# JuliaDiff/FiniteDiff.jl

Hardware: NVIDIA H100
Metric: jacobian_nnz_per_s (higher is better)
Workload: dtype f64

## Files before the change

finitediff.jl_b200/csrc/common.cuh:

```cuda
#pragma once
#include <cuda_runtime.h>
#include <stdint.h>

namespace fdb {

template <typename CT> struct ColorTraits;
template <> struct ColorTraits<uint8_t>  { static constexpr uint32_t invalid = 0xFFu; };
template <> struct ColorTraits<uint16_t> { static constexpr uint32_t invalid = 0xFFFFu; };
template <> struct ColorTraits<int32_t>  { static constexpr uint32_t invalid = 0x7FFFFFFFu; };

constexpr int kThreads = 256;

constexpr int kPairsPerThread = 2;
constexpr int kTile = kThreads * 2 * kPairsPerThread;

__device__ __forceinline__ double ld_stream(const double *p) { return __ldcs(p); }
__device__ __forceinline__ void st_stream(double *p, double v) { __stcs(p, v); }
__device__ __forceinline__ double2 ld_stream2(const double *p) { return __ldcs(reinterpret_cast<const double2 *>(p)); }
__device__ __forceinline__ void st_stream2(double *p, double a, double b) {
  __stcs(reinterpret_cast<double2 *>(p), make_double2(a, b));
}

template <typename CT> __device__ __forceinline__ void ld_color_pair(const CT *p, uint32_t &a, uint32_t &b);
template <> __device__ __forceinline__ void ld_color_pair<uint8_t>(const uint8_t *p, uint32_t &a, uint32_t &b) {
  const uint16_t v = __ldcs(reinterpret_cast<const unsigned short *>(p));
  a = v & 0xFFu; b = v >> 8;
}
template <> __device__ __forceinline__ void ld_color_pair<uint16_t>(const uint16_t *p, uint32_t &a, uint32_t &b) {
  const uint32_t v = __ldcs(reinterpret_cast<const unsigned int *>(p));
  a = v & 0xFFFFu; b = v >> 16;
}
template <> __device__ __forceinline__ void ld_color_pair<int32_t>(const int32_t *p, uint32_t &a, uint32_t &b) {
  const int2 v = __ldcs(reinterpret_cast<const int2 *>(p));
  a = (uint32_t)v.x; b = (uint32_t)v.y;
}

__device__ __forceinline__ double warp_sum(double v) {
#pragma unroll
  for (int o = 16; o > 0; o >>= 1) v += __shfl_xor_sync(0xffffffffu, v, o);
  return v;
}

}
```

finitediff.jl_b200/csrc/fdjac_abi.cu:

```cuda
#include "../../include/fdjac_b200.h"

#include <algorithm>
#include <climits>
#include <cstdarg>
#include <cmath>
#include <cfloat>
#include <cstdio>
#include <cstdlib>
#include <cstring>
#include <new>
#include <numeric>
#include <string>
#include <type_traits>
#include <vector>

#include <cub/device/device_radix_sort.cuh>
#include <cub/device/device_scan.cuh>

#include "common.cuh"
#include "kernels_eps.cuh"
#include "kernels_perturb.cuh"
#include "kernels_plan.cuh"
#include "kernels_scatter.cuh"
#include "kernels_staged.cuh"
#include "kernels_jvp.cuh"
#include "kernels_color.cuh"

using namespace fdb;

static thread_local std::string g_err;

static fdb_status fail(fdb_status st, const char *fmt, ...) {
  char buf[512];
  va_list ap;
  va_start(ap, fmt);
  vsnprintf(buf, sizeof buf, fmt, ap);
  va_end(ap);
  g_err = buf;
  return st;
}

#define CU(expr)                                                                                       \
  do {                                                                                                 \
    cudaError_t e__ = (expr);                                                                          \
    if (e__ != cudaSuccess)                                                                            \
      return fail(FDB_ERR_CUDA, "%s failed: %s (%s:%d)", #expr, cudaGetErrorString(e__), __FILE__, __LINE__); \
  } while (0)

#define TRY(expr)                    \
  do {                               \
    fdb_status s__ = (expr);         \
    if (s__ != FDB_OK) return s__;   \
  } while (0)

enum { SP_NONE = 0, SP_CSC = 1, SP_COO = 3, SP_BANDED = 4, SP_JVP = 5, SP_EPS = 6 };

struct DeviceGuard {
  int prev = -1;
  bool ok = false;
  explicit DeviceGuard(int dev) {
    if (cudaGetDevice(&prev) == cudaSuccess) {
      if (prev == dev) ok = true;
      else ok = cudaSetDevice(dev) == cudaSuccess;
    }
  }
  ~DeviceGuard() {
    int cur = -1;
    if (prev >= 0 && cudaGetDevice(&cur) == cudaSuccess && cur != prev) cudaSetDevice(prev);
  }
};

struct GraphKey {
  void *f = nullptr, *ctx = nullptr;
  const void *x = nullptr, *J = nullptr, *fx = nullptr, *f_in = nullptr;
  double relstep = 0, absstep = 0, dir = 0;
  int n_peers = 0;
  long long peer_generation = 0;
  const void *ext_eps = nullptr;
  bool operator==(const GraphKey &o) const {
    return f == o.f && ctx == o.ctx && x == o.x && J == o.J && fx == o.fx && f_in == o.f_in && relstep == o.relstep &&
           absstep == o.absstep && dir == o.dir && n_peers == o.n_peers && peer_generation == o.peer_generation &&
           ext_eps == o.ext_eps;
  }
};

struct fdb_plan {
  int device = 0, sm_count = 132;
  int64_t l2_bytes = 50 << 20;
  int fdtype = FDB_FORWARD, sp_kind = SP_CSC, jkind = FDB_J_CSC_NZVAL;
  int no_drift = 0;
  int rank = 0, world = 1;
  int64_t m = 0, n = 0, E = 0, j_len = 0, ldJ = 0, l = 0, u = 0;
  int32_t C = 0;
  int color_bits = 8;
  bool has_invalid = false;
  void *jcolor = nullptr;
  int32_t *row32 = nullptr;
  void *ecolor = nullptr;
  int64_t *dest = nullptr;
  int32_t *local_of = nullptr;
  int32_t *d_local_colors = nullptr;
  std::vector<int32_t> local_colors, owner;
  double *eps = nullptr, *sumsq = nullptr, *partial = nullptr;
  int eps_blocks = 0;
  int64_t eps_chunk = 0;
  int32_t eps_group = 1;
  const double *ext_eps = nullptr;
  unsigned int *ticket = nullptr;
  bool eps_lists = false;
  int64_t *bucket_start_d = nullptr, *chunk_base_d = nullptr;
  double *eps_list_partial = nullptr;
  int64_t eps_list_max_chunks = 0;
  bool peers_aligned = true;
  bool shared_J = false;
  double *fx_own = nullptr, *Fp = nullptr, *Fm = nullptr, *xp = nullptr, *xm = nullptr;
  int64_t slabs = 0, ldF = 0, ldx = 0, batch = 1, n_groups = 0;
  int64_t pbatch = 1;
  int strategy = 0;
  bool strategy_auto = true;
  bool lists_resident = false;
  struct Tunables {
    bool no_staged = false, no_eps_lists = false, no_eps_overlap = false, cm_prefetch = false, force_overlap = false;
    bool no_fx_cm = false, force_fx_cm = false, no_pack = false;
    int hi_stream = -1;
    int reverse = 3;
    int cm_slab_stream = 1;
    int eps_depth = 2;
    int cols_depth = 0, cols_gx = 64;
    int stages = 2;
    char staged_variant[3] = {'6', 'n', 0};
  } tune;
  bool double_buffer = false;
  cudaStream_t side = nullptr;
  cudaEvent_t ev_f[2] = {nullptr, nullptr}, ev_scat[2] = {nullptr, nullptr};
  cudaEvent_t ev_fork = nullptr, ev_eps = nullptr;
  int32_t *colptr32 = nullptr, *cols_by_color = nullptr;
  int32_t *cm_row = nullptr;
  void *cm_slot = nullptr;
  int64_t *cm_start = nullptr;
  double *fx_cm = nullptr;
  std::vector<int64_t> cm_start_h;
  int64_t cm_invalid_end = 0;
  uint16_t *row16 = nullptr;
  int32_t *tile_w0 = nullptr;
  int32_t stage_W = 0;
  bool staged = false, stage_packed = false;
  std::vector<int64_t> bucket_start;
  int lanes = 1;
  double mean_row_jump = 0.0;
  double **d_peers = nullptr;
  int n_peers = 0;
  int64_t col_begin = 0, col_end = 0;
  double *eps_cols = nullptr;
  cudaStream_t hstream = nullptr;
  double *h_dx = nullptr, *h_dJ = nullptr, *h_dfx = nullptr, *h_dfin = nullptr;
  std::vector<void *> allocs;
  size_t device_bytes = 0;
  fdb_counters_t cnt{};
  int64_t alg_bytes = 0;
  int64_t last_eps_count = 0;
  bool complex_entry = false;
  bool use_graph = false;
  cudaStream_t cstream = nullptr;
  cudaGraphExec_t graph_exec = nullptr;
  GraphKey graph_key;
  fdb_counters_t graph_delta{};
  long long peer_generation = 0;
  bool timing = false;
  std::vector<std::pair<cudaEvent_t, cudaEvent_t>> ev_pending, ev_pool;

  fdb_status alloc(void **p, size_t bytes) {
    if (bytes == 0) bytes = 16;
    cudaError_t e = cudaMalloc(p, bytes);
    if (e != cudaSuccess) {
      *p = nullptr;
      return fail(FDB_ERR_NOMEM, "cudaMalloc(%zu bytes) failed: %s", bytes, cudaGetErrorString(e));
    }
    allocs.push_back(*p);
    device_bytes += bytes;
    return FDB_OK;
  }
  template <typename T> fdb_status alloc_t(T **p, size_t count) { return alloc((void **)p, count * sizeof(T)); }
  int grid(int64_t items, int per_block = kThreads, int waves = 8) const {
    int64_t b = (items + per_block - 1) / per_block;
    const int64_t cap = (int64_t)sm_count * waves;
    if (b > cap) b = cap;
    if (b < 1) b = 1;
    return (int)b;
  }
};

struct I64View {
  const int64_t *d = nullptr;
  int64_t *owned = nullptr;
  ~I64View() { if (owned) cudaFree(owned); }
};

static fdb_status view_i64(const int64_t *p, int64_t count, I64View &v) {
  if (!p || count <= 0) { v.d = nullptr; return FDB_OK; }
  cudaPointerAttributes at{};
  cudaError_t e = cudaPointerGetAttributes(&at, p);
  if (e != cudaSuccess) { cudaGetLastError(); at.type = cudaMemoryTypeUnregistered; }
  if (at.type == cudaMemoryTypeDevice || at.type == cudaMemoryTypeManaged) { v.d = p; return FDB_OK; }
  CU(cudaMalloc((void **)&v.owned, (size_t)count * sizeof(int64_t)));
  CU(cudaMemcpy(v.owned, p, (size_t)count * sizeof(int64_t), cudaMemcpyHostToDevice));
  v.d = v.owned;
  return FDB_OK;
}

static fdb_status check_device(const fdb_plan_opts *o, int *dev) {
  int count = 0;
  cudaError_t e = cudaGetDeviceCount(&count);
  if (e != cudaSuccess || count <= 0) {
    cudaGetLastError();
    return fail(FDB_ERR_NO_DEVICE, "no CUDA device available (%s): libfdjac_b200 has no CPU fallback",
                e == cudaSuccess ? "device count 0" : cudaGetErrorString(e));
  }
  int d = 0;
  if (!o || o->use_current_device || o->device < 0) { CU(cudaGetDevice(&d)); }
  else d = o->device;
  if (d >= count) return fail(FDB_ERR_INVALID, "device %d out of range (%d devices)", d, count);
  *dev = d;
  return FDB_OK;
}

template <typename F> static fdb_status dispatch_ct(int bits, F &&fn) {
  if (bits == 8) return fn((uint8_t)0);
  if (bits == 16) return fn((uint16_t)0);
  return fn((int32_t)0);
}

static const char *plan_err_text(uint32_t e) {
  if (e & kErrColptr) return "colptr is not a valid CSC column pointer (must start at 1, be non-decreasing, end at nnz+1)";
  if (e & kErrRowRange) return "row index outside 1..m";
  if (e & kErrColRange) return "column index outside 1..n";
  if (e & kErrSlotRange) return "slot outside 1..j_len";
  if (e & kErrMissingInJ) return "a sparsity entry is absent from J's CSC pattern (the reference would insert a new stored entry; unsupported)";
  return "invalid pattern";
}

static fdb_status setup_colors(fdb_plan *P, const int64_t *colorvec , I64View &cv) {
  const int64_t n = P->n;
  TRY(view_i64(colorvec, n, cv));
  long long mx = n, mn = n > 0 ? 1 : 0;
  if (cv.d && n > 0) {
    long long *d_mm = nullptr;
    CU(cudaMalloc((void **)&d_mm, 2 * sizeof(long long)));
    long long init[2] = {LLONG_MIN, LLONG_MAX};
    CU(cudaMemcpy(d_mm, init, sizeof init, cudaMemcpyHostToDevice));
    color_minmax<<<P->grid(n), kThreads>>>(cv.d, n, d_mm, d_mm + 1);
    long long out[2];
    cudaError_t e = cudaMemcpy(out, d_mm, sizeof out, cudaMemcpyDeviceToHost);
    cudaFree(d_mm);
    if (e != cudaSuccess) return fail(FDB_ERR_CUDA, "colour min/max failed: %s", cudaGetErrorString(e));
    mx = out[0];
    mn = out[1];
  }
  if (n == 0) mx = 0;
  if (mx < 0) mx = 0;
  if (mx > 0x7FFFFFF0LL) return fail(FDB_ERR_UNSUPPORTED, "maximum(colorvec) = %lld exceeds 2^31", mx);
  P->C = (int32_t)mx;
  P->has_invalid = n > 0 && mn < 1;
  P->color_bits = mx <= 255 ? 8 : (mx <= 65535 ? 16 : 32);
  TRY(P->alloc(&P->jcolor, (size_t)std::max<int64_t>(n, 1) * (P->color_bits / 8)));
  if (n > 0) {
    uint32_t *d_flags = nullptr;
    const bool window_path = P->C > kEpsRegColors;
    if (window_path) {
      CU(cudaMalloc((void **)&d_flags, sizeof(uint32_t)));
      CU(cudaMemset(d_flags, 0, sizeof(uint32_t)));
    }
    fdb_status st = dispatch_ct(P->color_bits, [&](auto tag) -> fdb_status {
      using CT = decltype(tag);
      convert_colors<CT><<<P->grid(n), kThreads>>>(cv.d, n, (CT *)P->jcolor);
      if (window_path) color_lane_conflicts<CT><<<P->grid(n), kThreads>>>((const CT *)P->jcolor, n, P->C, d_flags);
      CU(cudaGetLastError());
      return FDB_OK;
    });
    if (st == FDB_OK && window_path) {
      uint32_t flags = 0;
      cudaError_t e = cudaMemcpy(&flags, d_flags, sizeof flags, cudaMemcpyDeviceToHost);
      if (e != cudaSuccess) st = fail(FDB_ERR_CUDA, "colour conflict flags: %s", cudaGetErrorString(e));
      P->eps_group = 1;
      for (int lg = 1; lg <= 5 && !(flags & (1u << lg)); ++lg) P->eps_group = 1 << lg;
    }
    if (d_flags) cudaFree(d_flags);
    if (st != FDB_OK) return st;
  }
  return FDB_OK;
}

static fdb_status alloc_eps_buffers(fdb_plan *P) {
  const int32_t C = P->C;
  TRY(P->alloc_t(&P->eps, std::max<int32_t>(C, 1)));
  TRY(P->alloc_t(&P->sumsq, std::max<int32_t>(C, 1)));
  {
    int64_t nb = (P->n + 2047) / 2048;
    nb = std::max<int64_t>(1, std::min<int64_t>(nb, (int64_t)P->sm_count * (C <= 256 ? 8 : 6)));
    P->eps_blocks = (int)nb;
    int64_t chunk = (P->n + nb - 1) / nb;
    P->eps_chunk = (std::max<int64_t>(chunk, 1) + 31) & ~(int64_t)31;
    const int64_t stride = C <= kEpsRegColors ? kEpsRegColors : std::min<int64_t>(C, kEpsWindow);
    TRY(P->alloc_t(&P->partial, (size_t)nb * stride));
    TRY(P->alloc_t(&P->ticket, 4));
    CU(cudaMemset(P->ticket, 0, 16));
  }

  return FDB_OK;
}

static fdb_status finish_colored_plan(fdb_plan *P, const fdb_plan_opts *o, const std::vector<unsigned long long> &count) {
  const int32_t C = P->C;
  P->owner.assign(C, 0);
  const int world = P->world;
  if (world > 1) {
    if (o && o->partition == 1) {
      std::vector<int32_t> order(C);
      std::iota(order.begin(), order.end(), 0);
      std::stable_sort(order.begin(), order.end(), [&](int32_t a, int32_t b) { return count[a] > count[b]; });
      std::vector<unsigned long long> load(world, 0);
      for (int32_t k : order) {
        int best = 0;
        for (int r = 1; r < world; ++r) if (load[r] < load[best]) best = r;
        P->owner[k] = best;
        load[best] += count[k] + 1;
      }
    } else {
      for (int32_t k = 0; k < C; ++k) P->owner[k] = k % world;
    }
  }
  std::vector<int32_t> local_of(C, -1);
  P->local_colors.clear();
  for (int32_t k = 0; k < C; ++k)
    if (P->owner[k] == P->rank) { local_of[k] = (int32_t)P->local_colors.size(); P->local_colors.push_back(k); }
  const int64_t n_local = (int64_t)P->local_colors.size();
  TRY(P->alloc_t(&P->local_of, std::max<int32_t>(C, 1)));
  TRY(P->alloc_t(&P->d_local_colors, std::max<int64_t>(n_local, 1)));
  if (C > 0) CU(cudaMemcpy(P->local_of, local_of.data(), (size_t)C * 4, cudaMemcpyHostToDevice));
  if (n_local > 0) CU(cudaMemcpy(P->d_local_colors, P->local_colors.data(), (size_t)n_local * 4, cudaMemcpyHostToDevice));

  TRY(alloc_eps_buffers(P));

  const bool central = P->fdtype == FDB_CENTRAL;
  const int64_t cw = P->fdtype == FDB_COMPLEX ? 2 : 1;
  P->ldF = (P->m + 1) & ~(int64_t)1;
  P->ldx = (P->n + 1) & ~(int64_t)1;
  if (P->ldF < 2) P->ldF = 2;
  if (P->ldx < 2) P->ldx = 2;
  int64_t budget = (o && o->scratch_bytes > 0) ? o->scratch_bytes : (int64_t)8 << 30;
  const int64_t per_slab = 8 * cw * P->ldF * (central ? 2 : 1);
  int64_t slabs = std::max<int64_t>(1, budget / per_slab);
  slabs = std::min<int64_t>(slabs, std::max<int64_t>(n_local, 1));
  if (P->sp_kind == SP_CSC && P->strategy == 0 && P->strategy_auto && slabs < n_local) P->strategy = 1;
  if (P->strategy == 1 && !P->lists_resident) {
    const int64_t l2_slabs = std::max<int64_t>(1, P->l2_bytes * 2 / 5 / per_slab);
    slabs = std::min<int64_t>(slabs, l2_slabs);
  }
  if (P->strategy == 1) slabs = std::min<int64_t>(slabs, kCmMaxGroup);
  P->slabs = slabs;
  P->n_groups = n_local == 0 ? 0 : (n_local + slabs - 1) / slabs;
  int64_t batch = (o && o->max_batch > 1) ? o->max_batch : 1;
  batch = std::min<int64_t>(batch, slabs);
  P->batch = batch;
  int64_t pbatch = std::max<int64_t>(batch, std::min<int64_t>(kPerturbMaxPoints, std::max<int64_t>(n_local, 1)));
  while (pbatch > batch && pbatch * 8 * cw * P->ldx * (central ? 2 : 1) > budget / 8) --pbatch;
  P->pbatch = pbatch;
  P->double_buffer = false;
  if (P->tune.force_overlap && P->sp_kind == SP_CSC && P->strategy == 1 && (int64_t)P->local_colors.size() > slabs) P->double_buffer = true;
  const size_t nbuf = P->double_buffer ? 2 : 1;
  CU(cudaStreamCreateWithFlags(&P->side, cudaStreamNonBlocking));
  CU(cudaEventCreateWithFlags(&P->ev_fork, cudaEventDisableTiming));
  CU(cudaEventCreateWithFlags(&P->ev_eps, cudaEventDisableTiming));
  if (P->double_buffer) {
    for (int b = 0; b < 2; ++b) {
      CU(cudaEventCreateWithFlags(&P->ev_f[b], cudaEventDisableTiming));
      CU(cudaEventCreateWithFlags(&P->ev_scat[b], cudaEventDisableTiming));
    }
  }
  TRY(P->alloc_t(&P->fx_own, (size_t)P->ldF));
  TRY(P->alloc_t(&P->Fp, nbuf * (size_t)slabs * P->ldF * cw));
  TRY(P->alloc_t(&P->xp, (size_t)pbatch * P->ldx * cw));
  if (central) {
    TRY(P->alloc_t(&P->Fm, nbuf * (size_t)slabs * P->ldF));
    TRY(P->alloc_t(&P->xm, (size_t)pbatch * P->ldx));
  }
  return FDB_OK;
}

static fdb_status build_color_lists(fdb_plan *P) {
  const int64_t n = P->n;
  const int32_t C = P->C;
  if (!P->cols_by_color) TRY(P->alloc_t(&P->cols_by_color, (size_t)std::max<int64_t>(n, 1)));
  if (n > 0) {
    uint32_t *k_in = nullptr, *k_out = nullptr;
    int32_t *v_in = nullptr;
    void *d_tmp = nullptr;
    size_t tmp_bytes = 0;
    auto cleanup = [&]() { cudaFree(k_in); cudaFree(k_out); cudaFree(v_in); cudaFree(d_tmp); };
    cudaError_t e = cudaMalloc((void **)&k_in, (size_t)n * 4);
    if (e == cudaSuccess) e = cudaMalloc((void **)&k_out, (size_t)n * 4);
    if (e == cudaSuccess) e = cudaMalloc((void **)&v_in, (size_t)n * 4);
    if (e == cudaSuccess) {
      dispatch_ct(P->color_bits, [&](auto tag) -> fdb_status {
        using CT = decltype(tag);
        color_sort_keys<CT><<<P->grid(n), kThreads>>>((const CT *)P->jcolor, n, C, k_in, v_in);
        return FDB_OK;
      });
      int end_bit = 1;
      while (end_bit < 32 && ((uint64_t)1 << end_bit) <= (uint64_t)C) ++end_bit;
      e = cub::DeviceRadixSort::SortPairs(nullptr, tmp_bytes, k_in, k_out, v_in, P->cols_by_color, (int)n, 0, end_bit);
      if (e == cudaSuccess) e = cudaMalloc(&d_tmp, tmp_bytes ? tmp_bytes : 16);
      if (e == cudaSuccess) e = cub::DeviceRadixSort::SortPairs(d_tmp, tmp_bytes, k_in, k_out, v_in, P->cols_by_color, (int)n, 0, end_bit);
      if (e == cudaSuccess) e = cudaDeviceSynchronize();
    }
    cleanup();
    if (e != cudaSuccess) return fail(FDB_ERR_CUDA, "column lists: %s", cudaGetErrorString(e));
  }
  if (C > kEpsRegColors && C <= (1 << 22) && n > 0) {
    std::vector<int64_t> cb((size_t)C + 1, 0);
    int64_t maxc = 1;
    for (int32_t k = 0; k < C; ++k) {
      const int64_t len = P->bucket_start[(size_t)k + 1] - P->bucket_start[(size_t)k];
      const int64_t nc = (len + kEpsListChunk - 1) / kEpsListChunk;
      cb[(size_t)k + 1] = cb[(size_t)k] + nc;
      maxc = std::max(maxc, nc);
    }
    TRY(P->alloc_t(&P->bucket_start_d, (size_t)C + 2));
    TRY(P->alloc_t(&P->chunk_base_d, (size_t)C + 1));
    TRY(P->alloc_t(&P->eps_list_partial, (size_t)std::max<int64_t>(cb[(size_t)C], 1)));
    CU(cudaMemcpy(P->bucket_start_d, P->bucket_start.data(), ((size_t)C + 2) * 8, cudaMemcpyHostToDevice));
    CU(cudaMemcpy(P->chunk_base_d, cb.data(), ((size_t)C + 1) * 8, cudaMemcpyHostToDevice));
    P->eps_list_max_chunks = maxc;
    P->eps_lists = true;
  }
  return FDB_OK;
}

static fdb_status bucket_offsets(fdb_plan *P, const unsigned long long *d_bucket_counts) {
  const int32_t C = P->C;
  std::vector<unsigned long long> bc((size_t)C + 1, 0);
  CU(cudaMemcpy(bc.data(), d_bucket_counts, ((size_t)C + 1) * 8, cudaMemcpyDeviceToHost));
  P->bucket_start.assign((size_t)C + 2, 0);
  for (int32_t k = 0; k <= C; ++k) P->bucket_start[(size_t)k + 1] = P->bucket_start[(size_t)k] + (int64_t)bc[(size_t)k];
  return FDB_OK;
}

__global__ void __launch_bounds__(kThreads)
cm_gather_cols(const int32_t *__restrict__ cols_by_color, const int64_t *__restrict__ src_start ,
               const int64_t *__restrict__ dst_start , int64_t nseg, int32_t *__restrict__ list_cols) {
  for (int64_t sgm = blockIdx.x; sgm < nseg; sgm += gridDim.x) {
    const int64_t s0 = src_start[sgm], d0 = dst_start[sgm], cnt = dst_start[sgm + 1] - d0;
    for (int64_t i = threadIdx.x; i < cnt; i += kThreads) list_cols[d0 + i] = cols_by_color[s0 + i];
  }
}

static fdb_status build_cm_lists(fdb_plan *P, const std::vector<unsigned long long> &count ) {
  const int64_t n_local = (int64_t)P->local_colors.size();
  const int32_t C = P->C;
  const bool zero_bucket = P->rank == 0 && P->bucket_start[(size_t)C + 1] > P->bucket_start[(size_t)C];
  const int64_t nseg = n_local + (zero_bucket ? 1 : 0);
  std::vector<int64_t> src(std::max<int64_t>(nseg, 1), 0), dst((size_t)nseg + 1, 0);
  P->cm_start_h.assign((size_t)n_local + 1, 0);
  unsigned long long valid_total = 0;
  for (int32_t k = 0; k < C; ++k) valid_total += count[(size_t)k];
  for (int64_t li = 0; li < n_local; ++li) {
    const int32_t k = P->local_colors[(size_t)li];
    src[(size_t)li] = P->bucket_start[(size_t)k];
    dst[(size_t)li + 1] = dst[(size_t)li] + (P->bucket_start[(size_t)k + 1] - P->bucket_start[(size_t)k]);
    P->cm_start_h[(size_t)li + 1] = P->cm_start_h[(size_t)li] + (int64_t)count[(size_t)k];
  }
  int64_t e_local = P->cm_start_h[(size_t)n_local];
  P->cm_invalid_end = e_local;
  if (zero_bucket) {
    src[(size_t)n_local] = P->bucket_start[(size_t)C];
    dst[(size_t)n_local + 1] = dst[(size_t)n_local] + (P->bucket_start[(size_t)C + 1] - P->bucket_start[(size_t)C]);
    e_local += P->E - (int64_t)valid_total;
    P->cm_invalid_end = e_local;
  }
  const int64_t ncols = dst[(size_t)nseg];
  TRY(P->alloc_t(&P->cm_start, (size_t)n_local + 1));
  CU(cudaMemcpy(P->cm_start, P->cm_start_h.data(), ((size_t)n_local + 1) * 8, cudaMemcpyHostToDevice));
  TRY(P->alloc_t(&P->cm_row, (size_t)std::max<int64_t>(e_local, 1)));
  {
    const bool want = P->n_groups > 1 || P->tune.force_fx_cm;
    if (P->fdtype == FDB_FORWARD && e_local > 0 && want && !P->tune.no_fx_cm) TRY(P->alloc_t(&P->fx_cm, (size_t)e_local));
  }
  const bool wide = P->dest != nullptr;
  TRY(P->alloc(&P->cm_slot, (size_t)std::max<int64_t>(e_local, 1) * (wide ? 8 : 4)));
  if (ncols == 0 || e_local == 0) return FDB_OK;
  int64_t *d_src = nullptr, *d_dst = nullptr;
  int32_t *list_cols = nullptr, *list_cnt = nullptr, *list_off = nullptr;
  void *d_tmp = nullptr;
  size_t tmp_bytes = 0;
  auto cleanup = [&]() {
    cudaFree(d_src); cudaFree(d_dst); cudaFree(list_cols); cudaFree(list_cnt); cudaFree(list_off); cudaFree(d_tmp);
  };
#define CM_CU(expr) do { cudaError_t e__ = (expr); if (e__ != cudaSuccess) { cleanup(); \
    return fail(FDB_ERR_CUDA, "%s failed: %s", #expr, cudaGetErrorString(e__)); } } while (0)
  CM_CU(cudaMalloc((void **)&d_src, (size_t)nseg * 8));
  CM_CU(cudaMalloc((void **)&d_dst, ((size_t)nseg + 1) * 8));
  CM_CU(cudaMalloc((void **)&list_cols, (size_t)ncols * 4));
  CM_CU(cudaMalloc((void **)&list_cnt, (size_t)ncols * 4));
  CM_CU(cudaMalloc((void **)&list_off, (size_t)ncols * 4));
  CM_CU(cudaMemcpy(d_src, src.data(), (size_t)nseg * 8, cudaMemcpyHostToDevice));
  CM_CU(cudaMemcpy(d_dst, dst.data(), ((size_t)nseg + 1) * 8, cudaMemcpyHostToDevice));
  cm_gather_cols<<<(int)std::min<int64_t>(nseg, (int64_t)P->sm_count * 16), kThreads>>>(P->cols_by_color, d_src, d_dst, nseg, list_cols);
  cm_column_counts<<<P->grid(ncols), kThreads>>>(list_cols, ncols, P->colptr32, list_cnt);
  CM_CU(cub::DeviceScan::ExclusiveSum(nullptr, tmp_bytes, list_cnt, list_off, (int)ncols));
  CM_CU(cudaMalloc(&d_tmp, tmp_bytes ? tmp_bytes : 16));
  CM_CU(cub::DeviceScan::ExclusiveSum(d_tmp, tmp_bytes, list_cnt, list_off, (int)ncols));
  {
    const int lanes = P->lanes;
    const int64_t blocks = (ncols + (kThreads / lanes) - 1) / (kThreads / lanes);
    const int grid = (int)std::max<int64_t>(1, std::min<int64_t>(blocks, (int64_t)P->sm_count * 16));
    if (wide) cm_expand<int64_t><<<grid, kThreads>>>(list_cols, list_off, ncols, P->colptr32, P->row32, P->dest, lanes, P->cm_row, (int64_t *)P->cm_slot);
    else cm_expand<int32_t><<<grid, kThreads>>>(list_cols, list_off, ncols, P->colptr32, P->row32, nullptr, lanes, P->cm_row, (int32_t *)P->cm_slot);
  }
  int32_t last_off = 0, last_cnt = 0;
  CM_CU(cudaMemcpy(&last_off, list_off + (ncols - 1), 4, cudaMemcpyDeviceToHost));
  CM_CU(cudaMemcpy(&last_cnt, list_cnt + (ncols - 1), 4, cudaMemcpyDeviceToHost));
  CM_CU(cudaDeviceSynchronize());
#undef CM_CU
  cleanup();
  if ((int64_t)last_off + last_cnt != e_local)
    return fail(FDB_ERR_INVALID, "internal: colour-major list holds %lld entries, expected %lld", (long long)last_off + last_cnt,
                (long long)e_local);
  return FDB_OK;
}

static fdb_status try_stage_plan(fdb_plan *P) {
  P->staged = false;
  if (P->tune.no_staged) return FDB_OK;
  if (P->sp_kind != SP_CSC || P->dest != nullptr || P->strategy != 0 || P->world != 1 || P->n_groups != 1) return FDB_OK;
  if (P->fdtype == FDB_COMPLEX || P->C < 1) return FDB_OK;
  const int nwin = P->fdtype == FDB_CENTRAL ? 2 * P->C : P->C + 1;
  const int64_t ntiles = P->E / kTile;
  if (nwin > kStageMaxWin || ntiles < 1) return FDB_OK;
  unsigned int *d_span = nullptr;
  TRY(P->alloc_t(&d_span, 1));
  CU(cudaMemset(d_span, 0, 4));
  TRY(P->alloc_t(&P->tile_w0, (size_t)ntiles));
  TRY(P->alloc_t(&P->row16, (size_t)ntiles * kTile));
  const int pgrid = (int)std::min<int64_t>(ntiles, (int64_t)P->sm_count * 16);
  stage_prepare<uint8_t><<<pgrid, kThreads>>>(P->row32, ntiles, P->tile_w0, P->row16, d_span, nullptr, P->C);
  unsigned int span = 0;
  CU(cudaMemcpy(&span, d_span, 4, cudaMemcpyDeviceToHost));
  const int64_t W = ((int64_t)span + 1) & ~(int64_t)1;
  P->stage_packed = P->C <= 14 && W <= 4096 && span > 0 && !P->tune.no_pack;
  if (P->stage_packed) {
    TRY(dispatch_ct(P->color_bits, [&](auto tag) -> fdb_status {
      using CT = decltype(tag);
      stage_prepare<CT><<<pgrid, kThreads>>>(P->row32, ntiles, P->tile_w0, P->row16, d_span, (const CT *)P->ecolor, P->C);
      CU(cudaGetLastError());
      return FDB_OK;
    }));
    CU(cudaDeviceSynchronize());
  }
  const size_t smem = (size_t)2 * nwin * W * 8 + 2 * kStagesMax * 8 + (size_t)P->C * 8;
  if (span == 0 || span > 65535 || smem > (size_t)kStageMaxSmem) return FDB_OK;
  P->stage_W = (int32_t)W;
  P->staged = true;
  return FDB_OK;
}

static fdb_status read_plan_err(uint32_t *d_err, const char *what) {
  uint32_t h = 0;
  CU(cudaMemcpy(&h, d_err, 4, cudaMemcpyDeviceToHost));
  const uint32_t hard = h & ~(uint32_t)(kErrPatternDiff | kErrRowOrder);
  if (hard == kErrMissingInJ) return fail(FDB_ERR_UNSUPPORTED, "%s: %s", what, plan_err_text(hard));
  if (hard) return fail(FDB_ERR_INVALID, "%s: %s", what, plan_err_text(hard));
  return FDB_OK;
}

static bool env_is(const char *name, char c) {
  const char *v = getenv(name);
  return v && v[0] == c;
}

static void read_tunables(fdb_plan *P) {
  auto &t = P->tune;
  t.no_staged = env_is("FDB_NO_STAGED", '1');
  t.no_eps_lists = env_is("FDB_NO_EPS_LISTS", '1');
  t.no_eps_overlap = env_is("FDB_NO_EPS_OVERLAP", '1');
  t.cm_prefetch = env_is("FDB_CM_PREFETCH", '1');
  t.force_overlap = env_is("FDB_FORCE_OVERLAP", '1');
  t.no_fx_cm = env_is("FDB_NO_FX_CM", '1');
  t.force_fx_cm = env_is("FDB_FORCE_FX_CM", '1');
  t.no_pack = env_is("FDB_NO_PACK", '1');
  if (const char *hs = getenv("FDB_HI_STREAM")) t.hi_stream = hs[0] == '1' ? 1 : 0;
  if (const char *v = getenv("FDB_REVERSE")) { if (v[0] >= '0' && v[0] <= '3') t.reverse = v[0] - '0'; }
  if (env_is("FDB_CM_HINT", '0')) t.cm_slab_stream = 0;
  if (env_is("FDB_STAGES", '3')) t.stages = 3;
  if (env_is("FDB_EPS_DEPTH", '1')) t.eps_depth = 1;
  if (env_is("FDB_COLS_DEPTH", '4')) t.cols_depth = 4;
  if (env_is("FDB_COLS_DEPTH", '2')) t.cols_depth = 2;
  if (env_is("FDB_COLS_DEPTH", '1')) t.cols_depth = 1;
  if (const char *v = getenv("FDB_COLS_GX")) { const int g = atoi(v); if (g >= 1 && g <= 4096) t.cols_gx = g; }
  if (const char *v = getenv("FDB_STAGED_VARIANT")) {
    if (v[0]) { t.staged_variant[0] = v[0]; t.staged_variant[1] = v[1] ? v[1] : 'n'; }
  }
}

static fdb_status new_plan(fdb_plan **out, const fdb_plan_opts *o, int64_t m, int64_t n) {
  if (!out) return fail(FDB_ERR_INVALID, "plan output pointer is NULL");
  *out = nullptr;
  if (m < 0 || n < 0) return fail(FDB_ERR_INVALID, "negative dimensions m=%lld n=%lld", (long long)m, (long long)n);
  if (m > 0x7FFFFFF0LL || n > 0x7FFFFFF0LL) return fail(FDB_ERR_UNSUPPORTED, "m, n must be < 2^31");
  if (o && o->fdtype != FDB_FORWARD && o->fdtype != FDB_CENTRAL && o->fdtype != FDB_COMPLEX)
    return fail(FDB_ERR_UNSUPPORTED, "Unrecognized fdtype: valid values are forward (0), central (1) and complex (2)");
  int dev = 0;
  TRY(check_device(o, &dev));
  fdb_plan *P = new (std::nothrow) fdb_plan();
  if (!P) return fail(FDB_ERR_NOMEM, "out of host memory");
  P->device = dev;
  P->m = m;
  P->n = n;
  P->fdtype = o ? o->fdtype : FDB_FORWARD;
  P->no_drift = o ? o->no_drift : 0;
  P->use_graph = o && o->use_graph != 0;
  P->shared_J = o && o->shared_j != 0;
  read_tunables(P);
  P->world = (o && o->world > 1) ? o->world : 1;
  P->rank = (o && o->world > 1) ? o->rank : 0;
  if (P->rank < 0 || P->rank >= P->world) {
    const int bad_rank = P->rank, bad_world = P->world;
    delete P;
    return fail(FDB_ERR_INVALID, "rank %d outside world %d", bad_rank, bad_world);
  }
  cudaDeviceProp prop;
  cudaError_t e = cudaGetDeviceProperties(&prop, dev);
  if (e != cudaSuccess) { delete P; return fail(FDB_ERR_CUDA, "cudaGetDeviceProperties: %s", cudaGetErrorString(e)); }
  P->sm_count = prop.multiProcessorCount;
  P->l2_bytes = prop.l2CacheSize;
  *out = P;
  return FDB_OK;
}

static void free_plan(fdb_plan *P) {
  if (!P) return;
  DeviceGuard g(P->device);
  for (void *p : P->allocs) cudaFree(p);
  for (auto &ev : P->ev_pending) { cudaEventDestroy(ev.first); cudaEventDestroy(ev.second); }
  for (auto &ev : P->ev_pool) { cudaEventDestroy(ev.first); cudaEventDestroy(ev.second); }
  if (P->hstream) cudaStreamDestroy(P->hstream);
  if (P->side) cudaStreamDestroy(P->side);
  for (int b = 0; b < 2; ++b) { if (P->ev_f[b]) cudaEventDestroy(P->ev_f[b]); if (P->ev_scat[b]) cudaEventDestroy(P->ev_scat[b]); }
  if (P->ev_fork) cudaEventDestroy(P->ev_fork);
  if (P->ev_eps) cudaEventDestroy(P->ev_eps);
  if (P->graph_exec) cudaGraphExecDestroy(P->graph_exec);
  if (P->cstream) cudaStreamDestroy(P->cstream);
  delete P;
}

#define PLAN_TRY(expr)                                   \
  do {                                                   \
    fdb_status s__ = (expr);                             \
    if (s__ != FDB_OK) { free_plan(P); *plan = nullptr; return s__; } \
  } while (0)

static inline void resolve_steps(int fdtype, double &relstep, double &absstep) {
  if (std::isnan(relstep)) relstep = fdb_default_relstep(fdtype);
  if (std::isnan(absstep)) absstep = relstep;
}

extern "C" {

int fdb_abi_version(void) { return FDB_ABI_VERSION; }
const char *fdb_last_error(void) { return g_err.c_str(); }
int fdb_device_count(void) {
  int c = 0;
  if (cudaGetDeviceCount(&c) != cudaSuccess) { cudaGetLastError(); return 0; }
  return c;
}

double fdb_default_relstep(int fdtype) {
  if (fdtype == FDB_FORWARD) return sqrt(DBL_EPSILON);
  if (fdtype == FDB_CENTRAL) return cbrt(DBL_EPSILON);
  return 1.0;
}
double fdb_compute_epsilon(int fdtype, double x, double relstep, double absstep, double dir) {
  const double a = relstep * fabs(x);
  const double e = a > absstep ? a : absstep;
  return fdtype == FDB_FORWARD ? e * dir : e;
}

fdb_status fdb_plan_create_csc(fdb_plan **plan, int64_t m, int64_t n, const int64_t *colptr, const int64_t *rowval,
                               int jkind, const int64_t *j_colptr, const int64_t *j_rowval, int64_t ldJ,
                               const int64_t *colorvec, const fdb_plan_opts *opts) {
  fdb_plan *P = nullptr;
  TRY(new_plan(plan, opts, m, n));
  P = *plan;
  DeviceGuard g(P->device);
  if (!colptr) { free_plan(P); *plan = nullptr; return fail(FDB_ERR_INVALID, "colptr is NULL"); }
  if (jkind != FDB_J_CSC_NZVAL && jkind != FDB_J_DENSE) {
    free_plan(P); *plan = nullptr;
    return fail(FDB_ERR_INVALID, "CSC sparsity supports J kinds CSC_NZVAL and DENSE");
  }
  P->sp_kind = SP_CSC;
  P->jkind = jkind;
  I64View cp, rv, cv, jcp, jrv;
  PLAN_TRY(view_i64(colptr, n + 1, cp));
  int64_t last = 1;
  {
    cudaError_t e = cudaMemcpy(&last, cp.d + n, 8, cudaMemcpyDeviceToHost);
    if (e != cudaSuccess) { free_plan(P); *plan = nullptr; return fail(FDB_ERR_CUDA, "reading colptr[n]: %s", cudaGetErrorString(e)); }
  }
  const int64_t nnz = last - 1;
  if (nnz < 0 || nnz > 0x7FFFFFF0LL) { free_plan(P); *plan = nullptr; return fail(FDB_ERR_UNSUPPORTED, "nnz=%lld unsupported (must be in [0, 2^31))", (long long)nnz); }
  if (nnz > 0 && !rowval) { free_plan(P); *plan = nullptr; return fail(FDB_ERR_INVALID, "rowval is NULL"); }
  P->E = nnz;
  PLAN_TRY(view_i64(rowval, nnz, rv));
  PLAN_TRY(setup_colors(P, colorvec, cv));

  uint32_t *d_err = nullptr;
  unsigned long long *d_cnt = nullptr;
  PLAN_TRY(P->alloc_t(&d_err, 1));
  PLAN_TRY(P->alloc_t(&d_cnt, std::max<int32_t>(P->C, 1)));
  cudaMemset(d_err, 0, 4);
  cudaMemset(d_cnt, 0, (size_t)std::max<int32_t>(P->C, 1) * 8);
  PLAN_TRY(P->alloc_t(&P->row32, std::max<int64_t>(nnz, 4)));
  PLAN_TRY(P->alloc(&P->ecolor, (size_t)std::max<int64_t>(nnz, 4) * (P->color_bits / 8) + 16));

  bool same_pattern = true;
  bool other_csc = false;
  if (jkind == FDB_J_CSC_NZVAL && j_colptr && j_rowval && (j_colptr != colptr || j_rowval != rowval)) {
    PLAN_TRY(view_i64(j_colptr, n + 1, jcp));
    int64_t jlast = 1;
    {
      cudaError_t e = cudaMemcpy(&jlast, jcp.d + n, 8, cudaMemcpyDeviceToHost);
      if (e != cudaSuccess) { free_plan(P); *plan = nullptr; return fail(FDB_ERR_CUDA, "reading J.colptr[n]: %s", cudaGetErrorString(e)); }
    }
    if (jlast < 1 || jlast - 1 > 0x7FFFFFF0LL) { free_plan(P); *plan = nullptr; return fail(FDB_ERR_INVALID, "J.colptr[n+1]=%lld is not a valid CSC end pointer", (long long)jlast); }
    const int64_t jnnz = jlast - 1;
    PLAN_TRY(view_i64(j_rowval, jnnz, jrv));
    if (jnnz != nnz) same_pattern = false;
    else {
      compare_i64<<<P->grid(n + 1), kThreads>>>(cp.d, jcp.d, n + 1, d_err);
      if (nnz > 0) compare_i64<<<P->grid(nnz), kThreads>>>(rv.d, jrv.d, nnz, d_err);
      uint32_t h = 0;
      cudaMemcpy(&h, d_err, 4, cudaMemcpyDeviceToHost);
      same_pattern = !(h & kErrPatternDiff);
      cudaMemset(d_err, 0, 4);
    }
    other_csc = !same_pattern;
    P->j_len = jnnz;
  } else if (jkind == FDB_J_CSC_NZVAL) {
    P->j_len = nnz;
  } else {
    if (ldJ < m) { free_plan(P); *plan = nullptr; return fail(FDB_ERR_INVALID, "ldJ=%lld < m=%lld", (long long)ldJ, (long long)m); }
    P->ldJ = ldJ;
    P->j_len = ldJ * n;
  }
  const bool need_dest = jkind == FDB_J_DENSE || other_csc;
  int32_t *col32 = nullptr;
  if (need_dest) {
    PLAN_TRY(P->alloc_t(&col32, std::max<int64_t>(nnz, 1)));
    PLAN_TRY(P->alloc_t(&P->dest, std::max<int64_t>(nnz, 1)));
  }
  validate_colptr<<<P->grid(n + 1), kThreads>>>(cp.d, n, nnz, d_err);
  PLAN_TRY(read_plan_err(d_err, "CSC sparsity"));
  if (other_csc) {
    validate_colptr<<<P->grid(n + 1), kThreads>>>(jcp.d, n, P->j_len, d_err);
    PLAN_TRY(read_plan_err(d_err, "J's CSC pattern"));
  }
  if (nnz > 0) {
    PLAN_TRY(dispatch_ct(P->color_bits, [&](auto tag) -> fdb_status {
      using CT = decltype(tag);
      const size_t hsm = P->C <= kPlanSmemColors ? (size_t)std::max<int32_t>(P->C, 1) * sizeof(unsigned int) : 0;
      expand_csc<CT><<<P->grid(nnz), kThreads, hsm>>>(cp.d, rv.d, m, n, nnz, (const CT *)P->jcolor, P->C, P->row32,
                                                 (CT *)P->ecolor, col32, d_cnt, d_err);
      CU(cudaGetLastError());
      return FDB_OK;
    }));
    if (jkind == FDB_J_DENSE) dest_dense_from_rc<<<P->grid(nnz), kThreads>>>(P->row32, col32, nnz, ldJ, P->dest);
    else if (other_csc) dest_other_csc<<<P->grid(nnz), kThreads>>>(P->row32, col32, nnz, jcp.d, jrv.d, P->dest, d_err);
  }
  PLAN_TRY(read_plan_err(d_err, "CSC sparsity"));
  std::vector<unsigned long long> cnt(std::max<int32_t>(P->C, 1), 0);
  if (P->C > 0) {
    cudaError_t e = cudaMemcpy(cnt.data(), d_cnt, (size_t)P->C * 8, cudaMemcpyDeviceToHost);
    if (e != cudaSuccess) { free_plan(P); *plan = nullptr; return fail(FDB_ERR_CUDA, "colour counts: %s", cudaGetErrorString(e)); }
  }
  {
    const int32_t C = P->C;
    unsigned long long *d_bucket = nullptr, *d_jump = nullptr;
    PLAN_TRY(P->alloc_t(&d_bucket, (size_t)C + 2));
    PLAN_TRY(P->alloc_t(&d_jump, 1));
    cudaMemset(d_bucket, 0, ((size_t)C + 2) * 8);
    cudaMemset(d_jump, 0, 8);
    PLAN_TRY(P->alloc_t(&P->colptr32, (size_t)n + 1));
    PLAN_TRY(P->alloc_t(&P->cols_by_color, (size_t)std::max<int64_t>(n, 1)));
    PLAN_TRY(dispatch_ct(P->color_bits, [&](auto tag) -> fdb_status {
      using CT = decltype(tag);
      colptr32_and_count<CT><<<P->grid(n + 1), kThreads>>>(cp.d, n, (const CT *)P->jcolor, C, P->colptr32, d_bucket);
      CU(cudaGetLastError());
      return FDB_OK;
    }));
    std::vector<unsigned long long> bc((size_t)C + 1, 0);
    {
      cudaError_t e = cudaMemcpy(bc.data(), d_bucket, ((size_t)C + 1) * 8, cudaMemcpyDeviceToHost);
      if (e != cudaSuccess) { free_plan(P); *plan = nullptr; return fail(FDB_ERR_CUDA, "column buckets: %s", cudaGetErrorString(e)); }
    }
    P->bucket_start.assign((size_t)C + 2, 0);
    for (int32_t k = 0; k <= C; ++k) P->bucket_start[(size_t)k + 1] = P->bucket_start[(size_t)k] + (int64_t)bc[(size_t)k];
    PLAN_TRY(build_color_lists(P));
    if (nnz > 1) {
      row_jump_sum<<<P->grid(nnz), kThreads>>>(P->row32, nnz, d_jump);
      unsigned long long js = 0;
      cudaMemcpy(&js, d_jump, 8, cudaMemcpyDeviceToHost);
      P->mean_row_jump = (double)js / (double)(nnz - 1);
    }
    int lanes = 1;
    const double avg = n > 0 ? (double)nnz / (double)n : 1.0;
    while (lanes < 32 && lanes < avg) lanes *= 2;
    P->lanes = lanes;
    const int want = opts ? opts->strategy : 0;
    bool per_color = P->world > 1;
    if (want == 1) per_color = false;
    if (want == 2 || want == 3) per_color = true;
    P->lists_resident = want == 3;
    if (want == 0 && P->world == 1 && P->mean_row_jump > 4096.0 && C >= 16 && 16 * P->m <= P->l2_bytes) {
      per_color = true;
      P->lists_resident = true;
    }
    P->strategy = per_color ? 1 : 0;
    P->strategy_auto = want == 0;
  }
  PLAN_TRY(finish_colored_plan(P, opts, cnt));
  if (P->strategy == 1) PLAN_TRY(build_cm_lists(P, cnt));
  PLAN_TRY(try_stage_plan(P));
  P->alg_bytes = 32 * nnz + 16 * n + 8;
  {
    cudaError_t e = cudaDeviceSynchronize();
    if (e != cudaSuccess) { free_plan(P); *plan = nullptr; return fail(FDB_ERR_CUDA, "plan build: %s", cudaGetErrorString(e)); }
  }
  return FDB_OK;
}

fdb_status fdb_plan_create_coo(fdb_plan **plan, int64_t m, int64_t n, int64_t nnz, const int64_t *rows_index,
                               const int64_t *cols_index, int jkind, const int64_t *slots, int64_t ldJ_or_jlen,
                               const int64_t *colorvec, const fdb_plan_opts *opts) {
  fdb_plan *P = nullptr;
  TRY(new_plan(plan, opts, m, n));
  P = *plan;
  DeviceGuard g(P->device);
  if (nnz < 0 || nnz > 0x7FFFFFF0LL) { free_plan(P); *plan = nullptr; return fail(FDB_ERR_UNSUPPORTED, "nnz=%lld unsupported", (long long)nnz); }
  if (nnz > 0 && (!rows_index || !cols_index)) { free_plan(P); *plan = nullptr; return fail(FDB_ERR_INVALID, "rows_index/cols_index NULL"); }
  if (jkind != FDB_J_DENSE && jkind != FDB_J_SLOTS) { free_plan(P); *plan = nullptr; return fail(FDB_ERR_INVALID, "COO sparsity supports J kinds DENSE and SLOTS"); }
  if (jkind == FDB_J_SLOTS && nnz > 0 && !slots) { free_plan(P); *plan = nullptr; return fail(FDB_ERR_INVALID, "slots is NULL"); }
  if (jkind == FDB_J_DENSE && ldJ_or_jlen < m) { free_plan(P); *plan = nullptr; return fail(FDB_ERR_INVALID, "ldJ < m"); }
  P->sp_kind = SP_COO;
  P->jkind = jkind;
  P->E = nnz;
  if (jkind == FDB_J_DENSE) { P->ldJ = ldJ_or_jlen; P->j_len = ldJ_or_jlen * n; }
  else P->j_len = ldJ_or_jlen;
  I64View rv, cvw, sv, cv;
  PLAN_TRY(view_i64(rows_index, nnz, rv));
  PLAN_TRY(view_i64(cols_index, nnz, cvw));
  if (jkind == FDB_J_SLOTS) PLAN_TRY(view_i64(slots, nnz, sv));
  PLAN_TRY(setup_colors(P, colorvec, cv));
  uint32_t *d_err = nullptr;
  unsigned long long *d_cnt = nullptr;
  PLAN_TRY(P->alloc_t(&d_err, 1));
  PLAN_TRY(P->alloc_t(&d_cnt, std::max<int32_t>(P->C, 1)));
  cudaMemset(d_err, 0, 4);
  cudaMemset(d_cnt, 0, (size_t)std::max<int32_t>(P->C, 1) * 8);
  PLAN_TRY(P->alloc_t(&P->row32, std::max<int64_t>(nnz, 4)));
  PLAN_TRY(P->alloc(&P->ecolor, (size_t)std::max<int64_t>(nnz, 4) * (P->color_bits / 8) + 16));
  PLAN_TRY(P->alloc_t(&P->dest, std::max<int64_t>(nnz, 1)));
  if (nnz > 0) {
    PLAN_TRY(dispatch_ct(P->color_bits, [&](auto tag) -> fdb_status {
      using CT = decltype(tag);
      const size_t hsm = P->C <= kPlanSmemColors ? (size_t)std::max<int32_t>(P->C, 1) * sizeof(unsigned int) : 0;
      prepare_coo<CT><<<P->grid(nnz), kThreads, hsm>>>(rv.d, cvw.d, jkind == FDB_J_SLOTS ? sv.d : nullptr, nnz, m, n, P->ldJ,
                                                  P->j_len, (const CT *)P->jcolor, P->C, P->row32, (CT *)P->ecolor,
                                                  P->dest, d_cnt, d_err);
      CU(cudaGetLastError());
      return FDB_OK;
    }));
  }
  PLAN_TRY(read_plan_err(d_err, "COO sparsity"));
  std::vector<unsigned long long> cnt(std::max<int32_t>(P->C, 1), 0);
  if (P->C > 0) cudaMemcpy(cnt.data(), d_cnt, (size_t)P->C * 8, cudaMemcpyDeviceToHost);
  PLAN_TRY(finish_colored_plan(P, opts, cnt));
  P->alg_bytes = 32 * nnz + 16 * n + 8;
  cudaError_t e = cudaDeviceSynchronize();
  if (e != cudaSuccess) { free_plan(P); *plan = nullptr; return fail(FDB_ERR_CUDA, "plan build: %s", cudaGetErrorString(e)); }
  return FDB_OK;
}

fdb_status fdb_plan_create_banded(fdb_plan **plan, int64_t m, int64_t n, int64_t l, int64_t u, int jkind, int64_t ldJ,
                                  const int64_t *colorvec, const fdb_plan_opts *opts) {
  fdb_plan *P = nullptr;
  TRY(new_plan(plan, opts, m, n));
  P = *plan;
  DeviceGuard g(P->device);
  if (jkind != FDB_J_BAND && jkind != FDB_J_DENSE) { free_plan(P); *plan = nullptr; return fail(FDB_ERR_INVALID, "banded sparsity supports J kinds BAND and DENSE"); }
  if (l + u + 1 < 1 || l < -n || u < -m) { free_plan(P); *plan = nullptr; return fail(FDB_ERR_INVALID, "invalid bandwidths l=%lld u=%lld", (long long)l, (long long)u); }
  if (jkind == FDB_J_DENSE && ldJ < m) { free_plan(P); *plan = nullptr; return fail(FDB_ERR_INVALID, "ldJ < m"); }
  P->sp_kind = SP_BANDED;
  P->jkind = jkind;
  P->l = l;
  P->u = u;
  P->ldJ = ldJ;
  P->j_len = jkind == FDB_J_BAND ? (l + u + 1) * n : ldJ * n;
  I64View cv;
  PLAN_TRY(setup_colors(P, colorvec, cv));
  unsigned long long *d_cnt = nullptr;
  PLAN_TRY(P->alloc_t(&d_cnt, std::max<int32_t>(P->C, 1)));
  cudaMemset(d_cnt, 0, (size_t)std::max<int32_t>(P->C, 1) * 8);
  if (n > 0 && P->C > 0) {
    PLAN_TRY(dispatch_ct(P->color_bits, [&](auto tag) -> fdb_status {
      using CT = decltype(tag);
      count_band_colors<CT><<<P->grid(n), kThreads>>>((const CT *)P->jcolor, m, n, l, u, P->C, d_cnt);
      CU(cudaGetLastError());
      return FDB_OK;
    }));
  }
  std::vector<unsigned long long> cnt(std::max<int32_t>(P->C, 1), 0);
  if (P->C > 0) cudaMemcpy(cnt.data(), d_cnt, (size_t)P->C * 8, cudaMemcpyDeviceToHost);
  unsigned long long total = 0;
  for (auto c : cnt) total += c;
  P->E = (int64_t)total;
  PLAN_TRY(finish_colored_plan(P, opts, cnt));
  P->alg_bytes = 8 * (int64_t)total + 16 * m * (int64_t)P->C;
  cudaError_t e = cudaDeviceSynchronize();
  if (e != cudaSuccess) { free_plan(P); *plan = nullptr; return fail(FDB_ERR_CUDA, "plan build: %s", cudaGetErrorString(e)); }
  return FDB_OK;
}

static fdb_status create_dense(fdb_plan **plan, int64_t m, int64_t n, int64_t ldJ, int64_t ncols, const fdb_plan_opts *opts) {
  fdb_plan *P = nullptr;
  TRY(new_plan(plan, opts, m, n));
  P = *plan;
  DeviceGuard g(P->device);
  if (ldJ < m) { free_plan(P); *plan = nullptr; return fail(FDB_ERR_INVALID, "ldJ < m"); }
  P->sp_kind = SP_NONE;
  P->jkind = FDB_J_DENSE;
  P->ldJ = ldJ;
  const int64_t per = (ncols + P->world - 1) / P->world;
  P->col_begin = std::min<int64_t>(ncols, per * P->rank);
  P->col_end = std::min<int64_t>(ncols, P->col_begin + per);
  const int64_t ncl = P->col_end - P->col_begin;
  P->j_len = ldJ * ncl;
  P->E = m * ncl;
  P->C = (int32_t)n;
  const bool central = P->fdtype == FDB_CENTRAL;
  P->ldF = std::max<int64_t>(2, (m + 1) & ~(int64_t)1);
  P->ldx = std::max<int64_t>(2, (n + 1) & ~(int64_t)1);
  int64_t batch = (opts && opts->max_batch > 1) ? opts->max_batch : 1;
  int64_t budget = (opts && opts->scratch_bytes > 0) ? opts->scratch_bytes : (int64_t)8 << 30;
  const int64_t cw = P->fdtype == FDB_COMPLEX ? 2 : 1;
  const int64_t per_point = 8 * cw * (P->ldx + P->ldF * (central ? 2 : 1));
  batch = std::max<int64_t>(1, std::min<int64_t>(batch, budget / per_point));
  batch = std::min<int64_t>(batch, std::max<int64_t>(ncl, 1));
  batch = std::min<int64_t>(batch, 65535);
  P->batch = batch;
  P->slabs = batch;
  P->n_groups = ncl == 0 ? 0 : (ncl + batch - 1) / batch;
  PLAN_TRY(P->alloc_t(&P->fx_own, (size_t)P->ldF));
  PLAN_TRY(P->alloc_t(&P->Fp, (size_t)batch * P->ldF * cw));
  if (central) PLAN_TRY(P->alloc_t(&P->Fm, (size_t)batch * P->ldF));
  PLAN_TRY(P->alloc_t(&P->xp, (size_t)batch * P->ldx * cw));
  PLAN_TRY(P->alloc_t(&P->eps_cols, (size_t)std::max<int64_t>(ncl, 1)));
  P->alg_bytes = 24 * m * ncl;
  return FDB_OK;
}

fdb_status fdb_plan_create_dense(fdb_plan **plan, int64_t m, int64_t n, int64_t ldJ, const fdb_plan_opts *opts) {
  return create_dense(plan, m, n, ldJ, n, opts);
}

fdb_status fdb_plan_create_dense_colorvec(fdb_plan **plan, int64_t m, int64_t n, int64_t ldJ, const int64_t *colorvec,
                                          const fdb_plan_opts *opts) {
  if (!plan) return fail(FDB_ERR_INVALID, "plan output pointer is NULL");
  *plan = nullptr;
  if (!colorvec) return create_dense(plan, m, n, ldJ, n, opts);
  if (n < 0 || m < 0) return fail(FDB_ERR_INVALID, "negative dimensions");
  int dev = 0;
  TRY(check_device(opts, &dev));
  DeviceGuard g(dev);
  long long mx = 0;
  if (n > 0) {
    I64View cv;
    TRY(view_i64(colorvec, n, cv));
    long long *d_mm = nullptr;
    CU(cudaMalloc((void **)&d_mm, 2 * sizeof(long long)));
    const long long init[2] = {LLONG_MIN, LLONG_MAX};
    cudaMemcpy(d_mm, init, sizeof init, cudaMemcpyHostToDevice);
    const int blocks = (int)std::max<int64_t>(1, std::min<int64_t>((n + kThreads - 1) / kThreads, 132 * 8));
    color_minmax<<<blocks, kThreads>>>(cv.d, n, d_mm, d_mm + 1);
    long long out[2] = {0, 0};
    const cudaError_t e = cudaMemcpy(out, d_mm, sizeof out, cudaMemcpyDeviceToHost);
    cudaFree(d_mm);
    if (e != cudaSuccess) return fail(FDB_ERR_CUDA, "colour maximum failed: %s", cudaGetErrorString(e));
    mx = out[0];
  }
  if (mx > n) return fail(FDB_ERR_INVALID, "sparsity=nothing: maximum(colorvec)=%lld indexes x beyond length(x)=%lld "
                                           "(BoundsError in the reference, jacobians.jl:549)", mx, (long long)n);
  return create_dense(plan, m, n, ldJ, mx < 0 ? 0 : (int64_t)mx, opts);
}

fdb_status fdb_plan_destroy(fdb_plan *plan) {
  free_plan(plan);
  return FDB_OK;
}

fdb_status fdb_plan_info(const fdb_plan *P, fdb_plan_info_t *info) {
  if (!P || !info) return fail(FDB_ERR_INVALID, "NULL argument");
  memset(info, 0, sizeof *info);
  info->m = P->m;
  info->n = P->n;
  info->n_entries = P->E;
  info->j_len = P->j_len;
  info->n_colors = P->C;
  const int64_t n_local = P->sp_kind == SP_NONE ? P->col_end - P->col_begin : (int64_t)P->local_colors.size();
  info->n_local_colors = n_local;
  info->n_groups = P->n_groups;
  info->slabs = P->slabs;
  info->fcalls_per_jacobian = P->fdtype == FDB_CENTRAL ? 2 * n_local : (P->fdtype == FDB_COMPLEX ? n_local : 1 + n_local);
  info->device_bytes = (int64_t)P->device_bytes;
  info->fdtype = P->fdtype;
  info->jkind = P->jkind;
  info->sp_kind = P->sp_kind;
  info->color_bits = P->color_bits;
  info->alg_bytes_scatter = P->alg_bytes;
  info->strategy = P->strategy;
  info->lanes = P->lanes;
  info->mean_row_jump = P->mean_row_jump;
  info->staged = P->staged ? 1 : 0;
  info->lists_resident = P->lists_resident ? 1 : 0;
  {
    const int64_t ct = P->color_bits / 8;
    const int64_t slabs_read = P->fdtype == FDB_CENTRAL ? 2 : 1;
    const int64_t fx_once = P->fdtype == FDB_FORWARD ? 8 * P->m : 0;
    if (P->sp_kind == SP_CSC || P->sp_kind == SP_COO) {
      if (P->sp_kind == SP_CSC && P->strategy == 1) {
        const int64_t e_local = P->cm_start_h.empty() ? 0 : P->cm_start_h.back();
        info->moved_bytes_scatter = e_local * (4 + (P->dest ? 8 : 4) + 8 * slabs_read + 8) + fx_once + (P->fx_cm ? e_local * (4 + 8 + 8) : 0);
      } else {
        const int64_t C = std::max<int32_t>(P->C, 1);
        const int64_t owned = P->world > 1 ? P->E * (int64_t)P->local_colors.size() / C : P->E;
        info->moved_bytes_scatter = P->E * (4 + ct) * std::max<int64_t>(P->n_groups, 1) + owned * (8 * slabs_read + 8 + (P->dest ? 8 : 0)) + fx_once;
        if (P->staged)
          info->moved_bytes_scatter = P->E * (2 + (P->stage_packed ? 0 : ct) + 8) + 8 * P->m * (int64_t)(P->fdtype == FDB_CENTRAL ? 2 * P->C : P->C + 1);
      }
    } else {
      info->moved_bytes_scatter = P->alg_bytes;
    }
  }
  return FDB_OK;
}

fdb_status fdb_plan_counters(const fdb_plan *P, fdb_counters_t *out) {
  if (!P || !out) return fail(FDB_ERR_INVALID, "NULL argument");
  *out = P->cnt;
  return FDB_OK;
}

fdb_status fdb_plan_dense_range(const fdb_plan *P, int64_t *b, int64_t *e) {
  if (!P || !b || !e) return fail(FDB_ERR_INVALID, "NULL argument");
  *b = P->col_begin;
  *e = P->col_end;
  return FDB_OK;
}

fdb_status fdb_plan_color_owner(const fdb_plan *P, int32_t *owner_out, int64_t cap) {
  if (!P || !owner_out) return fail(FDB_ERR_INVALID, "NULL argument");
  if (P->sp_kind == SP_NONE) return fail(FDB_ERR_INVALID, "dense plans partition columns by range");
  if (cap < (int64_t)P->owner.size()) return fail(FDB_ERR_INVALID, "owner_out too small");
  std::copy(P->owner.begin(), P->owner.end(), owner_out);
  return FDB_OK;
}

fdb_status fdb_plan_get_eps(fdb_plan *P, double *h_eps, int64_t cap, void *stream) {
  if (!P || !h_eps) return fail(FDB_ERR_INVALID, "NULL argument");
  DeviceGuard g(P->device);
  const int64_t count = P->sp_kind == SP_NONE ? P->col_end - P->col_begin : P->C;
  if (cap < count) return fail(FDB_ERR_INVALID, "h_eps too small (%lld < %lld)", (long long)cap, (long long)count);
  const double *src = P->sp_kind == SP_NONE ? P->eps_cols : P->eps;
  if (count > 0) {
    CU(cudaMemcpyAsync(h_eps, src, (size_t)count * 8, cudaMemcpyDeviceToHost, (cudaStream_t)stream));
    CU(cudaStreamSynchronize((cudaStream_t)stream));
  }
  return FDB_OK;
}

fdb_status fdb_plan_enable_timing(fdb_plan *P, int enable) {
  if (!P) return fail(FDB_ERR_INVALID, "NULL plan");
  P->timing = enable != 0;
  return FDB_OK;
}

fdb_status fdb_plan_read_timing(fdb_plan *P, double *scatter_ms, int64_t *scatter_launches) {
  if (!P || !scatter_ms || !scatter_launches) return fail(FDB_ERR_INVALID, "NULL argument");
  DeviceGuard g(P->device);
  double total = 0.0;
  int64_t count = 0;
  for (auto &ev : P->ev_pending) {
    CU(cudaEventSynchronize(ev.second));
    float ms = 0.f;
    CU(cudaEventElapsedTime(&ms, ev.first, ev.second));
    total += ms;
    count += 1;
    P->ev_pool.push_back(ev);
  }
  P->ev_pending.clear();
  *scatter_ms = total;
  *scatter_launches = count;
  return FDB_OK;
}

fdb_status fdb_plan_set_peers(fdb_plan *P, int n_peers, double *const *peer_J) {
  if (!P) return fail(FDB_ERR_INVALID, "NULL plan");
  if (n_peers < 0 || n_peers > 64) return fail(FDB_ERR_INVALID, "n_peers out of range");
  if (P->sp_kind == SP_NONE || P->sp_kind == SP_BANDED)
    return fail(FDB_ERR_UNSUPPORTED, "peer stores are implemented for the entry-driven (CSC / COO) scatters");
  DeviceGuard g(P->device);
  if (!P->d_peers) TRY(P->alloc_t(&P->d_peers, 64));
  if (n_peers > 0) CU(cudaMemcpy(P->d_peers, peer_J, (size_t)n_peers * sizeof(double *), cudaMemcpyHostToDevice));
  P->n_peers = n_peers;
  P->peer_generation += 1;
  P->peers_aligned = true;
  for (int i = 0; i < n_peers; ++i)
    if (reinterpret_cast<uintptr_t>(peer_J[i]) & 15) P->peers_aligned = false;
  return FDB_OK;
}

}

struct ScatterTimer {
  fdb_plan *P;
  cudaStream_t s;
  std::pair<cudaEvent_t, cudaEvent_t> ev{nullptr, nullptr};
  ScatterTimer(fdb_plan *p, cudaStream_t st) : P(p), s(st) {
    if (!P->timing) return;
    if (!P->ev_pool.empty()) { ev = P->ev_pool.back(); P->ev_pool.pop_back(); }
    else { cudaEventCreate(&ev.first); cudaEventCreate(&ev.second); }
    cudaEventRecord(ev.first, s);
  }
  ~ScatterTimer() {
    if (!P->timing || !ev.first) return;
    cudaEventRecord(ev.second, s);
    P->ev_pending.push_back(ev);
  }
};

static fdb_status zero_J(const fdb_plan *P, double *J, cudaStream_t s) {
  if (P->jkind == FDB_J_DENSE && P->ldJ > P->m) {
    const int64_t ncols = P->sp_kind == SP_NONE ? P->col_end - P->col_begin : P->n;
    if (P->m > 0 && ncols > 0)
      CU(cudaMemset2DAsync(J, (size_t)P->ldJ * 8, 0, (size_t)P->m * 8, (size_t)ncols, s));
    return FDB_OK;
  }
  CU(cudaMemsetAsync(J, 0, (size_t)P->j_len * 8, s));
  return FDB_OK;
}

static fdb_status call_f(fdb_plan *P, fdb_fn f, void *ctx, double *fx, const double *x, int64_t batch, cudaStream_t s) {
  const int rc = f(ctx, fx, x, batch, P->ldF, P->ldx, (void *)s);
  P->cnt.f_invocations += 1;
  P->cnt.f_points += batch;
  if (rc != 0) return fail(FDB_ERR_CALLBACK, "user f! returned %d", rc);
  return FDB_OK;
}

template <typename K>
static int resident_grid(const fdb_plan *P, K kernel, size_t dyn_smem, int64_t work_blocks) {
  int per_sm = 0;
  if (cudaOccupancyMaxActiveBlocksPerMultiprocessor(&per_sm, kernel, kThreads, dyn_smem) != cudaSuccess || per_sm < 1) {
    cudaGetLastError();
    per_sm = 4;
  }
  int64_t g = (int64_t)P->sm_count * per_sm;
  if (g > work_blocks) g = work_blocks;
  if (g < 1) g = 1;
  return (int)g;
}

template <typename CT>
static fdb_status run_eps(fdb_plan *P, const double *x, double relstep, double absstep, double dir, cudaStream_t s) {
  const int32_t C = P->C;
  if (C <= 0) return FDB_OK;
  if (P->fdtype == FDB_COMPLEX) {
    fill_value<<<(C + kThreads - 1) / kThreads, kThreads, 0, s>>>(P->eps, C, DBL_EPSILON);
    P->cnt.kernel_launches += 1;
    CU(cudaGetLastError());
    return FDB_OK;
  }
  EpsParams prm{P->fdtype == FDB_CENTRAL ? 1 : 0, relstep, absstep, dir};
  if (P->eps_lists) {
    if (!P->tune.no_eps_lists) {
      dim3 grid((unsigned)std::min<int64_t>(P->eps_list_max_chunks, 1024), (unsigned)std::min<int32_t>(C, 65535));
      color_sumsq_lists<<<grid, kThreads, 0, s>>>(x, P->cols_by_color, P->bucket_start_d, P->chunk_base_d, C, P->eps_list_partial);
      finalize_eps_lists<<<(int)std::min<int64_t>(((int64_t)C * 32 + kThreads - 1) / kThreads, (int64_t)P->sm_count * 8), kThreads, 0, s>>>(
          P->eps_list_partial, P->chunk_base_d, C, prm, P->eps, P->sumsq);
      P->cnt.kernel_launches += 2;
      CU(cudaGetLastError());
      return FDB_OK;
    }
  }
  if (C <= kEpsRegColors) {
    const int64_t ntiles = (P->n + kTile - 1) / kTile;
    const int aligned = (reinterpret_cast<uintptr_t>(x) & 15) == 0;
    auto go = [&](auto kern) {
      const int grid = std::min(resident_grid(P, kern, 0, ntiles), P->eps_blocks);
      kern<<<grid, kThreads, 0, s>>>(x, (const CT *)P->jcolor, P->n, aligned, C, prm, P->partial, P->ticket, P->eps, P->sumsq);
    };
    if (C <= 4) { if (P->tune.eps_depth == 2) go(color_sumsq_reg<CT, 4, 2>); else go(color_sumsq_reg<CT, 4, 1>); }
    else { if (P->tune.eps_depth == 2) go(color_sumsq_reg<CT, 8, 2>); else go(color_sumsq_reg<CT, 8, 1>); }
    P->cnt.kernel_launches += 1;
  } else {
    for (int32_t k0 = 0; k0 < C; k0 += kEpsWindow) {
      const int32_t W = std::min<int32_t>(kEpsWindow, C - k0);
      color_sumsq_win<CT><<<P->eps_blocks, kThreads, (size_t)kEpsWarps * W * sizeof(double), s>>>(
          x, (const CT *)P->jcolor, P->n, P->eps_chunk, k0, W, P->eps_group, P->partial);
      finalize_eps<<<(W * 32 + kThreads - 1) / kThreads, kThreads, 0, s>>>(P->partial, P->eps_blocks, W, k0, W, prm,
                                                                        P->eps, P->sumsq);
      P->cnt.kernel_launches += 2;
    }
  }
  CU(cudaGetLastError());
  return FDB_OK;
}

template <typename CT, int MODE>
static fdb_status run_colored(fdb_plan *P, fdb_fn f, void *ctx, const double *x, double *J, double *fx,
                              const double *f_in, double relstep, double absstep, double dir, cudaStream_t s) {
  constexpr bool CENTRAL = MODE == kCentral;
  constexpr bool COMPLEX = MODE == kComplex;
  const int64_t sF = COMPLEX ? 2 * P->ldF : P->ldF, sX = COMPLEX ? 2 * P->ldx : P->ldx;
  const int64_t n_local = (int64_t)P->local_colors.size();
  const bool ident = P->dest == nullptr && P->sp_kind != SP_BANDED;
  const bool band_data = P->sp_kind == SP_BANDED && P->jkind == FDB_J_BAND;
  const bool self_defining = (ident || band_data) && n_local > 0;
  if (!self_defining && P->n_peers == 0 && !P->shared_J && P->j_len > 0) TRY(zero_J(P, J, s));
  bool eps_beside_fx = MODE == kForward && !f_in && !P->ext_eps && P->side && P->ev_fork && P->C > 0;
  if (P->tune.no_eps_overlap) eps_beside_fx = false;
  if (P->ext_eps) {
    if (P->C > 0) CU(cudaMemcpyAsync(P->eps, P->ext_eps, (size_t)P->C * 8, cudaMemcpyDeviceToDevice, s));
  } else if (eps_beside_fx) {
    CU(cudaEventRecord(P->ev_fork, s));
    CU(cudaStreamWaitEvent(P->side, P->ev_fork, 0));
    TRY(run_eps<CT>(P, x, relstep, absstep, dir, P->side));
    CU(cudaEventRecord(P->ev_eps, P->side));
  } else {
    TRY(run_eps<CT>(P, x, relstep, absstep, dir, s));
  }
  const double *vfx = nullptr;
  if (MODE == kForward) {
    if (f_in) vfx = f_in;
    else { TRY(call_f(P, f, ctx, fx, x, 1, s)); vfx = fx; }
  }
  if (eps_beside_fx) CU(cudaStreamWaitEvent(s, P->ev_eps, 0));
  if (MODE == kForward && P->sp_kind == SP_CSC && P->strategy == 1 && P->fx_cm && n_local > 0) {
    const int64_t cnt = P->cm_start_h[(size_t)n_local];
    if (cnt > 0) {
      const int grid = (int)std::max<int64_t>(1, std::min<int64_t>((cnt + kThreads * 4 - 1) / (kThreads * 4), (int64_t)P->sm_count * 16));
      ScatterTimer tm(P, s);
      gather_fx_cm<<<grid, kThreads, 0, s>>>(P->cm_row, vfx, cnt, P->fx_cm);
      P->cnt.kernel_launches += 1;
    }
  }
  auto perturb_window = [&](int64_t li0, int64_t kc) -> fdb_status {
      for (int64_t q0 = 0; q0 < kc; q0 += kPerturbMaxPoints) {
        PerturbArgs pa{};
        pa.x = x; pa.jcolor = P->jcolor; pa.eps = P->eps;
        pa.xp = P->xp + q0 * sX; pa.xm = CENTRAL ? P->xm + q0 * sX : nullptr;
        pa.n = P->n; pa.ldx = sX; pa.C = P->C; pa.drift = P->no_drift ? 0 : 1;
        pa.reverse = (P->tune.reverse >> 1) & 1;
        pa.kcount = (int32_t)std::min<int64_t>(kPerturbMaxPoints, kc - q0);
        for (int32_t q = 0; q < pa.kcount; ++q) pa.k[q] = P->local_colors[(size_t)(li0 + q0 + q)];
        pa.aligned = ((reinterpret_cast<uintptr_t>(x) | reinterpret_cast<uintptr_t>(P->xp) |
                       reinterpret_cast<uintptr_t>(P->xm)) & 15) == 0 && (P->ldx & 1) == 0;
        const size_t sm = P->C <= kPerturbSmemColors ? (size_t)P->C * sizeof(double) : 0;
        const int64_t tiles = (P->n + kTile - 1) / kTile;
        if (COMPLEX) {
          if (pa.kcount == 1) perturb_complex<CT, 1><<<P->grid(P->n), kThreads, 0, s>>>(pa);
          else perturb_complex<CT, kPerturbMaxPoints><<<P->grid(P->n), kThreads, 0, s>>>(pa);
        } else {
          constexpr int kPerturbGridOver = 16;
          auto over = [&](int g) { return (int)std::max<int64_t>(1, std::min<int64_t>((int64_t)g * kPerturbGridOver, tiles)); };
          if (pa.kcount == 1)
            perturb_colors<CT, CENTRAL, 1><<<over(resident_grid(P, perturb_colors<CT, CENTRAL, 1>, sm, tiles)), kThreads, sm, s>>>(pa);
          else
            perturb_colors<CT, CENTRAL, kPerturbMaxPoints><<<over(resident_grid(P, perturb_colors<CT, CENTRAL, kPerturbMaxPoints>, sm, tiles)), kThreads, sm, s>>>(pa);
        }
        P->cnt.kernel_launches += 1;
      }
      return FDB_OK;
  };

  const bool overlap = P->double_buffer && P->side != nullptr;
  const double *Fp_g = P->Fp, *Fm_g = P->Fm;
  cudaStream_t ss = s;
  auto scatter_lists = [&](int64_t g, int64_t l0, int64_t G) -> fdb_status {
    const bool wide = P->dest != nullptr;
    if (g == 0 && P->rank == 0 && P->cm_invalid_end > P->cm_start_h[(size_t)n_local]) {
      const int64_t z0 = P->cm_start_h[(size_t)n_local], z1 = P->cm_invalid_end;
      const int grid = (int)std::max<int64_t>(1, std::min<int64_t>((z1 - z0 + kThreads - 1) / kThreads, (int64_t)P->sm_count * 8));
      if (wide) zero_slots<int64_t><<<grid, kThreads, 0, ss>>>(P->cm_slot, z0, z1, J, P->d_peers, P->n_peers);
      else zero_slots<int32_t><<<grid, kThreads, 0, ss>>>(P->cm_slot, z0, z1, J, P->d_peers, P->n_peers);
      P->cnt.kernel_launches += 1;
    }
    if (G <= 0) return FDB_OK;
    const int64_t total = P->cm_start_h[(size_t)(l0 + G)] - P->cm_start_h[(size_t)l0];
    if (total == 0) return FDB_OK;
    CmArgs a{};
    a.row = P->cm_row; a.slot = P->cm_slot; a.seg_start = P->cm_start; a.local_colors = P->d_local_colors;
    a.fx = vfx; a.Fp = Fp_g; a.Fm = Fm_g; a.eps = P->eps; a.J = J; a.peers = P->d_peers; a.n_peers = P->n_peers;
    a.fx_cm = MODE == kForward ? P->fx_cm : nullptr;
    a.l0 = (int32_t)l0; a.G = (int32_t)G; a.ldF = sF;
    a.m = COMPLEX ? 2 * P->m : P->m;
    a.prefetch_next = (G > 1 && P->tune.cm_prefetch) ? 1 : 0;
    a.slab_stream = P->tune.cm_slab_stream;
    const int64_t tiles = (total + kCmTile - 1) / kCmTile;
    ScatterTimer tm(P, ss);
    if (wide) {
      const int grid = resident_grid(P, diff_scatter_cm<MODE, int64_t>, 0, tiles);
      diff_scatter_cm<MODE, int64_t><<<grid, kThreads, 0, ss>>>(a);
    } else {
      const int grid = resident_grid(P, diff_scatter_cm<MODE, int32_t>, 0, tiles);
      diff_scatter_cm<MODE, int32_t><<<grid, kThreads, 0, ss>>>(a);
    }
    P->cnt.kernel_launches += 1;
    P->cnt.scatter_launches += 1;
    return FDB_OK;
  };

  auto scatter_group = [&](int64_t g, int64_t l0, int64_t G) -> fdb_status {
    if (P->sp_kind == SP_CSC && P->strategy == 1) return scatter_lists(g, l0, G);
    if (P->sp_kind == SP_BANDED) {
      BandArgs a{};
      ScatterTimer tm(P, s);
      a.jcolor = P->jcolor; a.fx = vfx; a.Fp = P->Fp; a.Fm = P->Fm; a.eps = P->eps; a.local_of = P->local_of;
      a.J = J; a.C = P->C; a.l0 = (int32_t)l0; a.G = (int32_t)G;
      a.write_other = (g == 0 && P->rank == 0) ? 1 : 0;
      a.to_dense = P->jkind == FDB_J_DENSE ? 1 : 0;
      a.ldF = sF; a.ldJ = P->ldJ; a.m = P->m; a.n = P->n; a.l = P->l; a.u = P->u;
      const int64_t w = P->l + P->u + 1;
      int64_t ntiles;
      a.cols_per_tile = std::max<int64_t>(1, 4096 / w);
      ntiles = (P->n + a.cols_per_tile - 1) / a.cols_per_tile;
      const bool prediv = !COMPLEX && w >= 64 && P->n > 0 && P->C > 0 && G > 0 && w >= 2 * (int64_t)P->C;
      if (prediv) {
        dim3 grid((unsigned)std::max(1, std::min(P->grid(P->m), std::max(1, P->sm_count * 8 / (int)G))), (unsigned)G);
        diff_slabs<MODE><<<grid, kThreads, 0, s>>>(P->Fp, CENTRAL ? P->Fm : vfx, P->eps, P->d_local_colors + l0, P->m, sF);
        P->cnt.kernel_launches += 1;
      }
      if (w >= 64 && P->n > 0) {
        const size_t sm = P->C <= kSmemTable ? (size_t)P->C * (sizeof(double) + sizeof(int32_t)) : 0;
        if (!a.to_dense && (reinterpret_cast<uintptr_t>(J) & 15) == 0) {
          const int32_t CH = (int32_t)std::min<int64_t>(2048, w & ~(int64_t)1);
          const int64_t nchunks = (w * P->n + CH - 1) / CH;
          if (prediv) {
            constexpr int kBandGridOver = 64;
            int grid = resident_grid(P, diff_scatter_band_flat<CT, kCopy>, sm, (nchunks + 7) / 8);
            grid = (int)std::max<int64_t>(1, std::min<int64_t>((int64_t)grid * kBandGridOver, (nchunks + 7) / 8));
            diff_scatter_band_flat<CT, kCopy><<<grid, kThreads, sm, s>>>(a, CH);
          } else {
            const int grid = resident_grid(P, diff_scatter_band_flat<CT, MODE>, sm, (nchunks + 7) / 8);
            diff_scatter_band_flat<CT, MODE><<<grid, kThreads, sm, s>>>(a, CH);
          }
        } else if (prediv) {
          const int grid = resident_grid(P, diff_scatter_band_wide<CT, kCopy>, sm, (P->n + 7) / 8);
          diff_scatter_band_wide<CT, kCopy><<<grid, kThreads, sm, s>>>(a);
        } else {
          const int grid = resident_grid(P, diff_scatter_band_wide<CT, MODE>, sm, (P->n + 7) / 8);
          diff_scatter_band_wide<CT, MODE><<<grid, kThreads, sm, s>>>(a);
        }
        P->cnt.kernel_launches += 1;
        P->cnt.scatter_launches += 1;
      } else if (ntiles > 0) {
        const int blocks = (int)std::min<int64_t>(ntiles, (int64_t)P->sm_count * 16);
        diff_scatter_band<CT, MODE><<<blocks, kThreads, 0, s>>>(a);
        P->cnt.kernel_launches += 1;
        P->cnt.scatter_launches += 1;
      }
    } else if (P->E > 0) {
      ScatterArgs a{};
      a.row = P->row32; a.ecolor = P->ecolor; a.dest = P->dest; a.fx = vfx; a.Fp = P->Fp; a.Fm = P->Fm; a.eps = P->eps;
      a.local_of = P->local_of; a.J = J; a.peers = P->d_peers; a.n_peers = P->n_peers; a.C = P->C;
      a.l0 = (int32_t)l0; a.G = (int32_t)G;
      a.write_invalid_zero = (g == 0 && P->rank == 0 && P->has_invalid) ? 1 : 0;
      a.ldF = sF; a.E = P->E;
      a.j_aligned = (reinterpret_cast<uintptr_t>(J) & 15) == 0 && P->peers_aligned;
      {
        a.hi_stream = P->tune.hi_stream >= 0 ? P->tune.hi_stream : (P->mean_row_jump > 4096.0 ? 1 : 0);
      }
      const size_t sm = P->C <= kSmemTable ? (size_t)P->C * (sizeof(double) + sizeof(int32_t)) : 0;
      ScatterTimer tm(P, s);
      if (ident) {
        const int64_t tiles = (P->E + kTile - 1) / kTile;
        const bool full = P->n_groups == 1 && P->world == 1 && P->n_peers == 0;
        bool staged = full && P->staged && MODE != kComplex;
        if (staged && MODE == kForward)
          staged = (reinterpret_cast<uintptr_t>(vfx) & 15) == 0 && ((P->m & 1) == 0 || vfx == P->fx_own);
        if (staged) {
          if constexpr (MODE != kComplex) {
            StagedArgs sa{};
            sa.row16 = P->row16; sa.ecolor = P->ecolor; sa.tile_w0 = P->tile_w0; sa.row32 = P->row32;
            sa.fx = vfx; sa.Fp = P->Fp; sa.Fm = P->Fm; sa.eps = P->eps; sa.J = J; sa.C = P->C; sa.W = P->stage_W;
            sa.ldF = sF; sa.src_len = P->ldF; sa.E = P->E; sa.j_aligned = a.j_aligned;
            sa.reverse = P->tune.reverse & 1;
            const int nwin = CENTRAL ? 2 * P->C : P->C + 1;
            int stages = P->tune.stages;
            if ((size_t)stages * nwin * P->stage_W * 8 + 2 * kStagesMax * 8 + (size_t)P->C * 8 > (size_t)kStageMaxSmem) stages = 2;
            sa.stages = stages;
            const size_t ssm = (size_t)stages * nwin * P->stage_W * 8 + 2 * kStagesMax * 8 + (size_t)P->C * 8;
            const char v0 = P->tune.staged_variant[0], v1 = P->tune.staged_variant[1];
            auto go = [&](auto kern) {
              const int grid = resident_grid(P, kern, ssm, tiles);
              kern<<<grid, kThreads, ssm, s>>>(sa);
            };
            if (P->stage_packed && v1 == 'e') go(diff_scatter_staged<CT, MODE, 6, false, true, true>);
            else if (P->stage_packed) go(diff_scatter_staged<CT, MODE, 6, false, true>);
            else if (v0 == '8') go(diff_scatter_staged<CT, MODE, 8, false, false>);
            else if (v1 == 'n') go(diff_scatter_staged<CT, MODE, 6, false, false>);
            else go(diff_scatter_staged<CT, MODE, 6, true, false>);
          }
        } else if (full) {
          const int grid = resident_grid(P, diff_scatter_ident<CT, MODE, true, kScatterMinBlocks>, sm, tiles);
          diff_scatter_ident<CT, MODE, true, kScatterMinBlocks><<<grid, kThreads, sm, s>>>(a);
        } else {
          const int grid = resident_grid(P, diff_scatter_ident<CT, MODE, false, kScatterMinBlocks>, sm, tiles);
          diff_scatter_ident<CT, MODE, false, kScatterMinBlocks><<<grid, kThreads, sm, s>>>(a);
        }
      } else {
        const int grid = resident_grid(P, diff_scatter_dest<CT, MODE>, sm, (P->E + kThreads - 1) / kThreads);
        diff_scatter_dest<CT, MODE><<<grid, kThreads, sm, s>>>(a);
      }
      P->cnt.kernel_launches += 1;
      P->cnt.scatter_launches += 1;
    }
    return FDB_OK;
  };

  int64_t li = 0;
  while (li < n_local) {
    const int64_t g = li / P->slabs, g0 = g * P->slabs, gend = std::min<int64_t>(g0 + P->slabs, n_local);
    if (li % P->pbatch == 0) TRY(perturb_window(li, std::min<int64_t>(P->pbatch, n_local - li)));
    const int64_t wend = std::min<int64_t>((li / P->pbatch + 1) * P->pbatch, n_local);
    const int64_t fc = std::min<int64_t>(P->batch, std::min<int64_t>(wend - li, gend - li));
    const int64_t gb = overlap ? (g & 1) * P->slabs * sF : 0;
    if (overlap && li == g0 && g >= 2) CU(cudaStreamWaitEvent(s, P->ev_scat[g & 1], 0));
    TRY(call_f(P, f, ctx, P->Fp + gb + (li - g0) * sF, P->xp + (li % P->pbatch) * sX, fc, s));
    if (CENTRAL) TRY(call_f(P, f, ctx, P->Fm + gb + (li - g0) * sF, P->xm + (li % P->pbatch) * sX, fc, s));
    li += fc;
    if (li == gend) {
      Fp_g = P->Fp + gb;
      Fm_g = CENTRAL ? P->Fm + gb : nullptr;
      if (overlap) {
        CU(cudaEventRecord(P->ev_f[g & 1], s));
        CU(cudaStreamWaitEvent(P->side, P->ev_f[g & 1], 0));
        ss = P->side;
        TRY(scatter_group(g, g0, gend - g0));
        CU(cudaEventRecord(P->ev_scat[g & 1], P->side));
        ss = s;
      } else {
        TRY(scatter_group(g, g0, gend - g0));
      }
    }
  }
  if (overlap) {
    const int64_t ng = (n_local + P->slabs - 1) / P->slabs;
    for (int64_t b = 0; b < std::min<int64_t>(ng, 2); ++b) CU(cudaStreamWaitEvent(s, P->ev_scat[b], 0));
  }
  if (n_local == 0 && P->sp_kind == SP_CSC && P->strategy == 1 && (P->n_peers > 0 || P->shared_J)) TRY(scatter_group(0, 0, 0));
  CU(cudaGetLastError());
  return FDB_OK;
}

template <int MODE>
static fdb_status run_dense(fdb_plan *P, fdb_fn f, void *ctx, const double *x, double *J, double *fx, const double *f_in,
                            double relstep, double absstep, double dir, cudaStream_t s) {
  constexpr bool CENTRAL = MODE == kCentral;
  constexpr bool COMPLEX = MODE == kComplex;
  const int64_t sF = COMPLEX ? 2 * P->ldF : P->ldF, sX = COMPLEX ? 2 * P->ldx : P->ldx;
  const int64_t ncl = P->col_end - P->col_begin;
  const double *vfx = nullptr;
  if (MODE == kForward) {
    if (f_in) vfx = f_in;
    else { TRY(call_f(P, f, ctx, fx, x, 1, s)); vfx = fx; }
  }
  if (ncl == 0) return FDB_OK;
  const int32_t B = (int32_t)P->batch;
  if (COMPLEX) {
    fill_value<<<(int)((ncl + kThreads - 1) / kThreads), kThreads, 0, s>>>(P->eps_cols, ncl, DBL_EPSILON);
    replicate_x_complex<<<P->grid(P->n), kThreads, 0, s>>>(x, P->n, sX, B, P->xp);
  } else {
    component_eps<<<(int)((ncl + kThreads - 1) / kThreads), kThreads, 0, s>>>(x, P->col_begin, ncl, CENTRAL ? 1 : 0, relstep,
                                                                            absstep, dir, P->eps_cols);
    replicate_x<<<P->grid(P->n), kThreads, 0, s>>>(x, P->n, P->ldx, B, P->xp);
  }
  P->cnt.kernel_launches += 2;
  int64_t prev_c0 = 0;
  int32_t prevB = 0;
  for (int64_t c0l = 0; c0l < ncl; c0l += B) {
    const int32_t kc = (int32_t)std::min<int64_t>(B, ncl - c0l);
    const int64_t c0 = P->col_begin + c0l;
    const int sb = (std::max(kc, prevB) + kThreads - 1) / kThreads;
    if (COMPLEX) set_components_complex<<<sb, kThreads, 0, s>>>(P->eps_cols, c0l, c0, prev_c0, kc, prevB, sX, P->xp);
    else set_components<<<sb, kThreads, 0, s>>>(x, P->eps_cols, c0l, c0, prev_c0, kc, prevB, P->ldx, 1.0, P->xp);
    TRY(call_f(P, f, ctx, P->Fp, P->xp, kc, s));
    if (CENTRAL) {
      set_components<<<sb, kThreads, 0, s>>>(x, P->eps_cols, c0l, c0, 0, kc, 0, P->ldx, -1.0, P->xp);
      TRY(call_f(P, f, ctx, P->Fm, P->xp, kc, s));
      P->cnt.kernel_launches += 1;
    }
    const int gx = (int)std::max<int64_t>(1, std::min<int64_t>((P->m / 2 + kThreads * 4 - 1) / (kThreads * 4), P->tune.cols_gx));
    dim3 grid((unsigned)gx, (unsigned)kc);
    {
      const double *lo_ptr = CENTRAL ? P->Fm : vfx;
      const int pairs_ok = ((reinterpret_cast<uintptr_t>(J + c0l * P->ldJ) | reinterpret_cast<uintptr_t>(lo_ptr) |
                             reinterpret_cast<uintptr_t>(P->Fp)) & 15) == 0 && (P->ldJ & 1) == 0 && (sF & 1) == 0;
      ScatterTimer tm(P, s);
      auto go = [&](auto kern) { kern<<<grid, kThreads, 0, s>>>(P->Fp, lo_ptr, P->eps_cols, c0l, kc, P->m, sF, P->ldJ, J + c0l * P->ldJ, pairs_ok); };
      const int depth = P->tune.cols_depth ? P->tune.cols_depth : (CENTRAL ? 4 : 2);
      if (depth == 4) go(diff_columns<MODE, 4>);
      else if (depth == 2) go(diff_columns<MODE, 2>);
      else go(diff_columns<MODE, 1>);
    }
    P->cnt.kernel_launches += 2;
    P->cnt.scatter_launches += 1;
    prev_c0 = c0;
    prevB = kc;
  }
  CU(cudaGetLastError());
  return FDB_OK;
}

extern "C" {

static fdb_status jacobian_eager(fdb_plan *P, fdb_fn f, void *ctx, const double *d_x, double *d_J, double *fx,
                                 const double *d_f_in, double relstep, double absstep, double dir, cudaStream_t s) {
  if (P->sp_kind == SP_NONE) {
    if (P->fdtype == FDB_CENTRAL) return run_dense<kCentral>(P, f, ctx, d_x, d_J, fx, d_f_in, relstep, absstep, dir, s);
    if (P->fdtype == FDB_COMPLEX) return run_dense<kComplex>(P, f, ctx, d_x, d_J, fx, d_f_in, relstep, absstep, dir, s);
    return run_dense<kForward>(P, f, ctx, d_x, d_J, fx, d_f_in, relstep, absstep, dir, s);
  }
  return dispatch_ct(P->color_bits, [&](auto tag) -> fdb_status {
    using CT = decltype(tag);
    if (P->fdtype == FDB_CENTRAL) return run_colored<CT, kCentral>(P, f, ctx, d_x, d_J, fx, d_f_in, relstep, absstep, dir, s);
    if (P->fdtype == FDB_COMPLEX) return run_colored<CT, kComplex>(P, f, ctx, d_x, d_J, fx, d_f_in, relstep, absstep, dir, s);
    return run_colored<CT, kForward>(P, f, ctx, d_x, d_J, fx, d_f_in, relstep, absstep, dir, s);
  });
}

fdb_status fdb_jacobian(fdb_plan *P, fdb_fn f, void *ctx, const double *d_x, double *d_J, double *d_fx,
                        const double *d_f_in, double relstep, double absstep, double dir, void *stream) {
  if (!P || !f) return fail(FDB_ERR_INVALID, "NULL plan or f");
  if ((P->n > 0 && !d_x) || (P->j_len > 0 && !d_J)) return fail(FDB_ERR_INVALID, "NULL x or J");
  if (P->sp_kind == SP_JVP) return fail(FDB_ERR_INVALID, "this is a JVP plan: call fdb_jvp");
  if (P->sp_kind == SP_EPS) return fail(FDB_ERR_INVALID, "this is a step-size plan: call fdb_color_eps");
  if (P->fdtype == FDB_COMPLEX && !P->complex_entry)
    return fail(FDB_ERR_INVALID, "this plan is a complex-step plan: call fdb_jacobian_complex with a complex128 callback");
  DeviceGuard g(P->device);
  if (!g.ok) return fail(FDB_ERR_CUDA, "cannot select device %d", P->device);
  cudaStream_t s = (cudaStream_t)stream;
  resolve_steps(P->fdtype, relstep, absstep);
  double *fx = d_fx ? d_fx : P->fx_own;
  fdb_status st;
  if (P->use_graph && !P->timing) {
    const GraphKey key{(void *)f, ctx, d_x, d_J, fx, d_f_in, relstep, absstep, dir, P->n_peers, P->peer_generation, P->ext_eps};
    if (!P->graph_exec || !(key == P->graph_key)) {
      if (P->graph_exec) { cudaGraphExecDestroy(P->graph_exec); P->graph_exec = nullptr; }
      if (!P->cstream) CU(cudaStreamCreateWithFlags(&P->cstream, cudaStreamNonBlocking));
      const fdb_counters_t before = P->cnt;
      CU(cudaStreamBeginCapture(P->cstream, cudaStreamCaptureModeThreadLocal));
      st = jacobian_eager(P, f, ctx, d_x, d_J, fx, d_f_in, relstep, absstep, dir, P->cstream);
      cudaGraph_t graph = nullptr;
      cudaError_t e = cudaStreamEndCapture(P->cstream, &graph);
      if (st != FDB_OK) { if (graph) cudaGraphDestroy(graph); cudaGetLastError(); return st; }
      if (e != cudaSuccess || !graph) {
        cudaGetLastError();
        return fail(FDB_ERR_CUDA, "stream capture of the Jacobian failed (%s): the f! callback must be capture-safe "
                                  "(enqueue-only, no allocation) when use_graph is set", cudaGetErrorString(e));
      }
      e = cudaGraphInstantiate(&P->graph_exec, graph, 0);
      cudaGraphDestroy(graph);
      if (e != cudaSuccess) { P->graph_exec = nullptr; return fail(FDB_ERR_CUDA, "cudaGraphInstantiate: %s", cudaGetErrorString(e)); }
      P->graph_key = key;
      P->graph_delta.f_points = P->cnt.f_points - before.f_points;
      P->graph_delta.f_invocations = P->cnt.f_invocations - before.f_invocations;
      P->graph_delta.kernel_launches = P->cnt.kernel_launches - before.kernel_launches;
      P->graph_delta.scatter_launches = P->cnt.scatter_launches - before.scatter_launches;
      P->cnt = before;
    }
    CU(cudaGraphLaunch(P->graph_exec, s));
    P->cnt.f_points += P->graph_delta.f_points;
    P->cnt.f_invocations += P->graph_delta.f_invocations;
    P->cnt.kernel_launches += P->graph_delta.kernel_launches;
    P->cnt.scatter_launches += P->graph_delta.scatter_launches;
    st = FDB_OK;
  } else {
    st = jacobian_eager(P, f, ctx, d_x, d_J, fx, d_f_in, relstep, absstep, dir, s);
  }
  if (st == FDB_OK) P->cnt.jacobians += 1;
  return st;
}

fdb_status fdb_jacobian_complex(fdb_plan *P, fdb_fn_c f, void *ctx, const double *d_x, double *d_J, void *stream) {
  if (!P || !f) return fail(FDB_ERR_INVALID, "NULL plan or f");
  if (P->fdtype != FDB_COMPLEX) return fail(FDB_ERR_INVALID, "fdb_jacobian_complex needs a plan created with fdtype = FDB_COMPLEX");
  P->complex_entry = true;
  const fdb_status st = fdb_jacobian(P, reinterpret_cast<fdb_fn>(f), ctx, d_x, d_J, nullptr, nullptr, FDB_STEP_DEFAULT, FDB_STEP_DEFAULT, 1.0, stream);
  P->complex_entry = false;
  return st;
}

fdb_status fdb_eps_plan_create(fdb_plan **plan, int64_t n, const int64_t *colorvec, const fdb_plan_opts *opts) {
  fdb_plan *P = nullptr;
  TRY(new_plan(plan, opts, 0, n));
  P = *plan;
  DeviceGuard g(P->device);
  P->sp_kind = SP_EPS;
  I64View cv;
  PLAN_TRY(setup_colors(P, colorvec, cv));
  PLAN_TRY(alloc_eps_buffers(P));
  if (P->C > kEpsRegColors && n > 0) {
    unsigned long long *d_bucket = nullptr;
    PLAN_TRY(P->alloc_t(&d_bucket, (size_t)P->C + 2));
    cudaMemset(d_bucket, 0, ((size_t)P->C + 2) * 8);
    PLAN_TRY(dispatch_ct(P->color_bits, [&](auto tag) -> fdb_status {
      using CT = decltype(tag);
      count_color_buckets<CT><<<P->grid(n), kThreads>>>((const CT *)P->jcolor, n, P->C, d_bucket);
      CU(cudaGetLastError());
      return FDB_OK;
    }));
    PLAN_TRY(bucket_offsets(P, d_bucket));
    PLAN_TRY(build_color_lists(P));
  }
  return FDB_OK;
}

fdb_status fdb_color_eps(fdb_plan *P, const double *d_x, double relstep, double absstep, double dir, double *d_eps_out,
                         void *stream) {
  if (!P) return fail(FDB_ERR_INVALID, "NULL plan");
  if (P->sp_kind == SP_NONE || P->sp_kind == SP_JVP) return fail(FDB_ERR_INVALID, "fdb_color_eps needs a coloured plan");
  if (P->n > 0 && !d_x) return fail(FDB_ERR_INVALID, "NULL x");
  DeviceGuard g(P->device);
  if (!g.ok) return fail(FDB_ERR_CUDA, "cannot select device %d", P->device);
  cudaStream_t s = (cudaStream_t)stream;
  resolve_steps(P->fdtype, relstep, absstep);
  TRY(dispatch_ct(P->color_bits, [&](auto tag) -> fdb_status {
    using CT = decltype(tag);
    return run_eps<CT>(P, d_x, relstep, absstep, dir, s);
  }));
  if (d_eps_out && P->C > 0) CU(cudaMemcpyAsync(d_eps_out, P->eps, (size_t)P->C * 8, cudaMemcpyDeviceToDevice, s));
  return FDB_OK;
}

fdb_status fdb_plan_set_external_eps(fdb_plan *P, const double *d_eps) {
  if (!P) return fail(FDB_ERR_INVALID, "NULL plan");
  if (P->sp_kind == SP_NONE || P->sp_kind == SP_JVP || P->sp_kind == SP_EPS)
    return fail(FDB_ERR_INVALID, "external step sizes apply to coloured Jacobian plans");
  P->ext_eps = d_eps;
  return FDB_OK;
}

fdb_status fdb_jvp_plan_create(fdb_plan **plan, int64_t m, int64_t n, const fdb_plan_opts *opts) {
  fdb_plan *P = nullptr;
  TRY(new_plan(plan, opts, m, n));
  P = *plan;
  DeviceGuard g(P->device);
  if (P->fdtype == FDB_COMPLEX) {
    free_plan(P); *plan = nullptr;
    return fail(FDB_ERR_UNSUPPORTED, "finite_difference_jvp doesn't support :complex-mode finite diff");
  }
  P->sp_kind = SP_JVP;
  P->C = 1;
  P->ldF = std::max<int64_t>(2, (m + 1) & ~(int64_t)1);
  P->ldx = std::max<int64_t>(2, (n + 1) & ~(int64_t)1);
  int64_t nb = std::max<int64_t>(1, std::min<int64_t>((n + kTile - 1) / kTile, (int64_t)P->sm_count * 8));
  P->eps_blocks = (int)nb;
  PLAN_TRY(P->alloc_t(&P->partial, (size_t)nb));
  PLAN_TRY(P->alloc_t(&P->ticket, 4));
  cudaMemset(P->ticket, 0, 16);
  PLAN_TRY(P->alloc_t(&P->eps, 2));
  PLAN_TRY(P->alloc_t(&P->sumsq, 2));
  PLAN_TRY(P->alloc_t(&P->fx_own, (size_t)P->ldF));
  PLAN_TRY(P->alloc_t(&P->xp, (size_t)P->ldx));
  P->alg_bytes = 24 * n + 24 * m;
  return FDB_OK;
}

fdb_status fdb_jvp(fdb_plan *P, fdb_fn f, void *ctx, double *d_jvp, const double *d_x, const double *d_v, double *d_x1,
                   double *d_fx1, const double *d_f_in, double relstep, double absstep, double dir, void *stream) {
  if (!P || !f) return fail(FDB_ERR_INVALID, "NULL plan or f");
  if (P->sp_kind != SP_JVP) return fail(FDB_ERR_INVALID, "not a JVP plan (fdb_jvp_plan_create)");
  if ((P->n > 0 && (!d_x || !d_v)) || (P->m > 0 && !d_jvp)) return fail(FDB_ERR_INVALID, "NULL jvp, x or v");
  DeviceGuard g(P->device);
  if (!g.ok) return fail(FDB_ERR_CUDA, "cannot select device %d", P->device);
  cudaStream_t s = (cudaStream_t)stream;
  resolve_steps(P->fdtype, relstep, absstep);
  double *x1 = d_x1 ? d_x1 : P->xp;
  double *fx1 = d_fx1 ? d_fx1 : P->fx_own;
  const bool central = P->fdtype == FDB_CENTRAL;
  const int64_t n = P->n, m = P->m;
  const int al_xv = ((reinterpret_cast<uintptr_t>(d_x) | reinterpret_cast<uintptr_t>(d_v)) & 15) == 0;
  const int al_x1 = al_xv && (reinterpret_cast<uintptr_t>(x1) & 15) == 0;
  EpsParams prm{central ? 1 : 0, relstep, absstep, dir};
  const int64_t tiles = (n + kTile - 1) / kTile;
  const int grid_n = std::min(resident_grid(P, jvp_dot_eps, 0, tiles), P->eps_blocks);
  jvp_dot_eps<<<grid_n, kThreads, 0, s>>>(d_x, d_v, n, al_xv, prm, P->partial, P->ticket, P->eps, P->sumsq);
  P->cnt.kernel_launches += 1;
  const double *base = fx1;
  if (!central) {
    if (d_f_in) base = d_f_in;
    else TRY(call_f(P, f, ctx, fx1, d_x, 1, s));
  } else {
    jvp_point<<<resident_grid(P, jvp_point, 0, tiles), kThreads, 0, s>>>(d_x, d_v, P->eps, 1, x1, n, al_x1);
    P->cnt.kernel_launches += 1;
    TRY(call_f(P, f, ctx, fx1, x1, 1, s));
  }
  jvp_point<<<resident_grid(P, jvp_point, 0, tiles), kThreads, 0, s>>>(d_x, d_v, P->eps, 0, x1, n, al_x1);
  TRY(call_f(P, f, ctx, d_jvp, x1, 1, s));
  jvp_quotient<<<P->grid(m), kThreads, 0, s>>>(d_jvp, base, P->eps, central ? 1 : 0, m);
  P->cnt.kernel_launches += 2;
  CU(cudaGetLastError());
  P->cnt.jacobians += 1;
  return FDB_OK;
}

fdb_status fdb_jacobian_host(fdb_plan *P, fdb_fn f, void *ctx, const double *h_x, double *h_J, double *h_fx,
                             const double *h_f_in, double relstep, double absstep, double dir) {
  if (!P || !f) return fail(FDB_ERR_INVALID, "NULL plan or f");
  if ((P->n > 0 && !h_x) || (P->j_len > 0 && !h_J)) return fail(FDB_ERR_INVALID, "NULL x or J");
  DeviceGuard g(P->device);
  if (!g.ok) return fail(FDB_ERR_CUDA, "cannot select device %d", P->device);
  if (!P->hstream) {
    CU(cudaStreamCreateWithFlags(&P->hstream, cudaStreamNonBlocking));
    TRY(P->alloc_t(&P->h_dx, (size_t)std::max<int64_t>(P->n, 1)));
    TRY(P->alloc_t(&P->h_dJ, (size_t)std::max<int64_t>(P->j_len, 1)));
    TRY(P->alloc_t(&P->h_dfx, (size_t)P->ldF));
    TRY(P->alloc_t(&P->h_dfin, (size_t)P->ldF));
  }
  cudaStream_t s = P->hstream;
  if (P->n > 0) CU(cudaMemcpyAsync(P->h_dx, h_x, (size_t)P->n * 8, cudaMemcpyHostToDevice, s));
  const double *fin = nullptr;
  if (h_f_in && P->fdtype == FDB_FORWARD) {
    CU(cudaMemcpyAsync(P->h_dfin, h_f_in, (size_t)P->m * 8, cudaMemcpyHostToDevice, s));
    fin = P->h_dfin;
  }
  fdb_status st = fdb_jacobian(P, f, ctx, P->h_dx, P->h_dJ, P->h_dfx, fin, relstep, absstep, dir, (void *)s);
  if (st != FDB_OK) { cudaStreamSynchronize(s); return st; }
  if (P->j_len > 0) {
    if (P->jkind == FDB_J_DENSE && P->ldJ > P->m) {
      const int64_t ncols = P->sp_kind == SP_NONE ? P->col_end - P->col_begin : P->n;
      if (P->m > 0 && ncols > 0)
        CU(cudaMemcpy2DAsync(h_J, (size_t)P->ldJ * 8, P->h_dJ, (size_t)P->ldJ * 8, (size_t)P->m * 8, (size_t)ncols,
                             cudaMemcpyDeviceToHost, s));
    } else {
      CU(cudaMemcpyAsync(h_J, P->h_dJ, (size_t)P->j_len * 8, cudaMemcpyDeviceToHost, s));
    }
  }
  if (h_fx && P->fdtype == FDB_FORWARD && !fin && P->m > 0)
    CU(cudaMemcpyAsync(h_fx, P->h_dfx, (size_t)P->m * 8, cudaMemcpyDeviceToHost, s));
  CU(cudaStreamSynchronize(s));
  return FDB_OK;
}

fdb_status fdb_host_alloc(void **p, size_t bytes) {
  if (!p) return fail(FDB_ERR_INVALID, "NULL argument");
  CU(cudaHostAlloc(p, bytes ? bytes : 16, cudaHostAllocDefault));
  return FDB_OK;
}
fdb_status fdb_host_free(void *p) { if (p) CU(cudaFreeHost(p)); return FDB_OK; }
fdb_status fdb_device_alloc(void **p, size_t bytes) {
  if (!p) return fail(FDB_ERR_INVALID, "NULL argument");
  CU(cudaMalloc(p, bytes ? bytes : 16));
  return FDB_OK;
}
fdb_status fdb_device_free(void *p) { if (p) CU(cudaFree(p)); return FDB_OK; }
fdb_status fdb_memcpy_h2d(void *d, const void *h, size_t bytes, void *stream) {
  CU(cudaMemcpyAsync(d, h, bytes, cudaMemcpyHostToDevice, (cudaStream_t)stream));
  return FDB_OK;
}
fdb_status fdb_memcpy_d2h(void *h, const void *d, size_t bytes, void *stream) {
  CU(cudaMemcpyAsync(h, d, bytes, cudaMemcpyDeviceToHost, (cudaStream_t)stream));
  return FDB_OK;
}
fdb_status fdb_stream_sync(void *stream) { CU(cudaStreamSynchronize((cudaStream_t)stream)); return FDB_OK; }

fdb_status fdb_ipc_get_handle(void *d_ptr, unsigned char handle[64]) {
  static_assert(sizeof(cudaIpcMemHandle_t) == 64, "CUDA IPC handle size");
  cudaIpcMemHandle_t h;
  CU(cudaIpcGetMemHandle(&h, d_ptr));
  memcpy(handle, &h, 64);
  return FDB_OK;
}
fdb_status fdb_ipc_open(const unsigned char handle[64], void **d_ptr) {
  cudaIpcMemHandle_t h;
  memcpy(&h, handle, 64);
  CU(cudaIpcOpenMemHandle(d_ptr, h, cudaIpcMemLazyEnablePeerAccess));
  return FDB_OK;
}
fdb_status fdb_ipc_close(void *d_ptr) { CU(cudaIpcCloseMemHandle(d_ptr)); return FDB_OK; }

}

#include "fdjac_group.cuh"
```

finitediff.jl_b200/csrc/kernels_eps.cuh:

```cuda
#pragma once
#include "common.cuh"

namespace fdb {

constexpr int kEpsRegColors = 8;
constexpr int kEpsWindow = 512;
constexpr int kEpsWarps = kThreads / 32;
constexpr int kEpsBatch = 4;

struct EpsParams {
  int fdtype_central;
  double relstep, absstep, dir;
};

__device__ __forceinline__ double eps_from_sumsq(double ss, const EpsParams &p) {
  const double tmp = sqrt(ss);
  const double a = p.relstep * fabs(sqrt(tmp));
  double e = a > p.absstep ? a : p.absstep;
  if (!p.fdtype_central) e = e * p.dir;
  return e;
}

template <int NC>
__device__ __forceinline__ void sumsq_accumulate(double (&acc)[NC], double v, uint32_t c) {
  const double sq = v * v;
#pragma unroll
  for (int k = 0; k < NC; ++k)
    if (c == (uint32_t)k) acc[k] += sq;
}

template <typename CT, int NC, int DEPTH = 1>
__global__ void __launch_bounds__(kThreads)
color_sumsq_reg(const double *__restrict__ x, const CT *__restrict__ jcolor, int64_t n, int x_aligned, int32_t C,
                EpsParams prm, double *__restrict__ partial ,
                unsigned int *__restrict__ ticket, double *__restrict__ eps, double *__restrict__ sumsq) {
  double acc[NC];
#pragma unroll
  for (int k = 0; k < NC; ++k) acc[k] = 0.0;
  constexpr int kHalf = kTile / 2;
  const int64_t nfull = x_aligned ? n / kTile : 0;
  const int tid2 = 2 * threadIdx.x;
  int64_t tile = blockIdx.x;
  if (DEPTH == 2) {
    for (; tile + gridDim.x < nfull; tile += 2 * (int64_t)gridDim.x) {
      const double *__restrict__ xa = x + tile * kTile, *__restrict__ xb = xa + (int64_t)gridDim.x * kTile;
      const CT *__restrict__ ca = jcolor + tile * kTile, *__restrict__ cb = ca + (int64_t)gridDim.x * kTile;
      const double2 a0 = ld_stream2(xa + tid2), a1 = ld_stream2(xa + kHalf + tid2);
      const double2 b0 = ld_stream2(xb + tid2), b1 = ld_stream2(xb + kHalf + tid2);
      uint32_t p0, p1, p2, p3, q0, q1, q2, q3;
      ld_color_pair<CT>(ca + tid2, p0, p1);
      ld_color_pair<CT>(ca + kHalf + tid2, p2, p3);
      ld_color_pair<CT>(cb + tid2, q0, q1);
      ld_color_pair<CT>(cb + kHalf + tid2, q2, q3);
      sumsq_accumulate<NC>(acc, a0.x, p0);
      sumsq_accumulate<NC>(acc, a0.y, p1);
      sumsq_accumulate<NC>(acc, a1.x, p2);
      sumsq_accumulate<NC>(acc, a1.y, p3);
      sumsq_accumulate<NC>(acc, b0.x, q0);
      sumsq_accumulate<NC>(acc, b0.y, q1);
      sumsq_accumulate<NC>(acc, b1.x, q2);
      sumsq_accumulate<NC>(acc, b1.y, q3);
    }
  }
  for (; tile < nfull; tile += gridDim.x) {
    const double *__restrict__ xt = x + tile * kTile;
    const CT *__restrict__ ct = jcolor + tile * kTile;
    const double2 va = ld_stream2(xt + tid2);
    const double2 vb = ld_stream2(xt + kHalf + tid2);
    uint32_t ca0, ca1, cb0, cb1;
    ld_color_pair<CT>(ct + tid2, ca0, ca1);
    ld_color_pair<CT>(ct + kHalf + tid2, cb0, cb1);
    sumsq_accumulate<NC>(acc, va.x, ca0);
    sumsq_accumulate<NC>(acc, va.y, ca1);
    sumsq_accumulate<NC>(acc, vb.x, cb0);
    sumsq_accumulate<NC>(acc, vb.y, cb1);
  }
  {
    const int64_t rem0 = nfull * kTile;
    const int64_t ntail = (n - rem0 + kTile - 1) / kTile;
    for (int64_t tt = blockIdx.x; tt < ntail; tt += gridDim.x) {
      const int64_t base = rem0 + tt * kTile;
#pragma unroll
      for (int u = 0; u < kPairsPerThread; ++u) {
        const int64_t j = base + u * kHalf + tid2;
        if (j < n) sumsq_accumulate<NC>(acc, ld_stream(x + j), (uint32_t)jcolor[j]);
        if (j + 1 < n) sumsq_accumulate<NC>(acc, ld_stream(x + j + 1), (uint32_t)jcolor[j + 1]);
      }
    }
  }
  __shared__ double s[kEpsWarps][kEpsRegColors];
  __shared__ bool s_last;
  const int lane = threadIdx.x & 31, w = threadIdx.x >> 5;
#pragma unroll
  for (int k = 0; k < NC; ++k) {
    const double t = warp_sum(acc[k]);
    if (lane == 0) s[w][k] = t;
  }
  __syncthreads();
  if (threadIdx.x < NC) {
    double t = 0.0;
#pragma unroll
    for (int ww = 0; ww < kEpsWarps; ++ww) t += s[ww][threadIdx.x];
    __stcg(partial + (int64_t)blockIdx.x * kEpsRegColors + threadIdx.x, t);
  }
  __threadfence();
  __syncthreads();
  if (threadIdx.x == 0) s_last = atomicAdd(ticket, 1u) == gridDim.x - 1;
  __syncthreads();
  if (!s_last) return;
  static_assert(kEpsWarps == kEpsRegColors, "one warp per register colour");
  if (w < C) {
    double t0 = 0.0, t1 = 0.0, t2 = 0.0, t3 = 0.0;
    int b = lane;
    for (; b + 96 < (int)gridDim.x; b += 128) {
      t0 += __ldcg(partial + (int64_t)b * kEpsRegColors + w);
      t1 += __ldcg(partial + (int64_t)(b + 32) * kEpsRegColors + w);
      t2 += __ldcg(partial + (int64_t)(b + 64) * kEpsRegColors + w);
      t3 += __ldcg(partial + (int64_t)(b + 96) * kEpsRegColors + w);
    }
    for (; b < (int)gridDim.x; b += 32) t0 += __ldcg(partial + (int64_t)b * kEpsRegColors + w);
    double t = warp_sum((t0 + t1) + (t2 + t3));
    if (lane == 0) {
      eps[w] = eps_from_sumsq(t, prm);
      if (sumsq) sumsq[w] = t;
    }
  }
  if (threadIdx.x == 0) *ticket = 0u;
}

template <typename CT>
__global__ void __launch_bounds__(kThreads)
color_sumsq_win(const double *__restrict__ x, const CT *__restrict__ jcolor, int64_t n, int64_t chunk, int32_t k0,
                int32_t W, int32_t group, double *__restrict__ partial ) {
  extern __shared__ double sacc[];
  for (int i = threadIdx.x; i < kEpsWarps * W; i += kThreads) sacc[i] = 0.0;
  __syncthreads();
  const int lane = threadIdx.x & 31, w = threadIdx.x >> 5;
  double *acc = sacc + (size_t)w * W;
  const int64_t start = (int64_t)blockIdx.x * chunk;
  int64_t end = start + chunk;
  if (end > n) end = n;
  constexpr int64_t kStep = (int64_t)kEpsWarps * 32;
  const int my_group = lane / (group > 0 ? group : 1);
  for (int64_t base = start + (int64_t)w * 32; base < end; base += kStep * kEpsBatch) {
    double v[kEpsBatch];
    int32_t cc[kEpsBatch];
#pragma unroll
    for (int u = 0; u < kEpsBatch; ++u) {
      const int64_t j = base + u * kStep + lane;
      v[u] = 0.0;
      cc[u] = -1;
      if (j < end) {
        v[u] = ld_stream(x + j);
        cc[u] = (int32_t)(uint32_t)jcolor[j] - k0;
      }
    }
#pragma unroll
    for (int u = 0; u < kEpsBatch; ++u) {
      const int32_t c = (cc[u] >= 0 && cc[u] < W) ? cc[u] : -1;
      const double sq = v[u] * v[u];
      if (group == 32) {
        if (c >= 0) acc[c] += sq;
        __syncwarp();
      } else if (group >= 4) {
        for (int ph = 0; ph < 32 / group; ++ph) {
          if (c >= 0 && my_group == ph) acc[c] += sq;
          __syncwarp();
        }
      } else {
        const unsigned act = __ballot_sync(0xffffffffu, c >= 0);
        if (c >= 0) {
          const unsigned peers = __match_any_sync(act, c);
          double s = 0.0;
          unsigned mm = peers;
          while (mm) {
            const int l = __ffs(mm) - 1;
            mm &= mm - 1;
            s += __shfl_sync(peers, sq, l);
          }
          if (lane == __ffs(peers) - 1) acc[c] += s;
        }
        __syncwarp();
      }
    }
  }
  __syncthreads();
  for (int i = threadIdx.x; i < W; i += kThreads) {
    double t = 0.0;
#pragma unroll
    for (int ww = 0; ww < kEpsWarps; ++ww) t += sacc[(size_t)ww * W + i];
    partial[(int64_t)blockIdx.x * W + i] = t;
  }
}

constexpr int kEpsListChunk = 4096;

__global__ void __launch_bounds__(kThreads)
color_sumsq_lists(const double *__restrict__ x, const int32_t *__restrict__ cols_by_color,
                  const int64_t *__restrict__ bucket_start , const int64_t *__restrict__ chunk_base ,
                  int32_t C, double *__restrict__ partial) {
  __shared__ double s[kEpsWarps];
  for (int32_t k = blockIdx.y; k < C; k += gridDim.y) {
    const int64_t b0 = bucket_start[k], len = bucket_start[k + 1] - b0;
    const int64_t nchunks = (len + kEpsListChunk - 1) / kEpsListChunk;
    for (int64_t ch = blockIdx.x; ch < nchunks; ch += gridDim.x) {
      const int64_t c0 = b0 + ch * kEpsListChunk;
      int64_t c1 = c0 + kEpsListChunk;
      if (c1 > b0 + len) c1 = b0 + len;
      double v[kEpsListChunk / kThreads];
#pragma unroll
      for (int u = 0; u < kEpsListChunk / kThreads; ++u) {
        const int64_t i = c0 + u * kThreads + threadIdx.x;
        v[u] = i < c1 ? __ldg(x + __ldcs(cols_by_color + i)) : 0.0;
      }
      double acc = 0.0;
#pragma unroll
      for (int u = 0; u < kEpsListChunk / kThreads; ++u) acc += v[u] * v[u];
      acc = warp_sum(acc);
      if ((threadIdx.x & 31) == 0) s[threadIdx.x >> 5] = acc;
      __syncthreads();
      if (threadIdx.x == 0) {
        double t = 0.0;
#pragma unroll
        for (int w = 0; w < kEpsWarps; ++w) t += s[w];
        partial[chunk_base[k] + ch] = t;
      }
      __syncthreads();
    }
  }
}

__global__ void __launch_bounds__(kThreads)
finalize_eps_lists(const double *__restrict__ partial, const int64_t *__restrict__ chunk_base, int32_t C, EpsParams prm,
                   double *__restrict__ eps, double *__restrict__ sumsq) {
  const int lane = threadIdx.x & 31;
  const int64_t warp = (blockIdx.x * (int64_t)kThreads + threadIdx.x) >> 5;
  const int64_t nwarps = ((int64_t)gridDim.x * kThreads) >> 5;
  for (int64_t k = warp; k < C; k += nwarps) {
    const int64_t p0 = chunk_base[k], p1 = chunk_base[k + 1];
    double t = 0.0;
    for (int64_t p = p0 + lane; p < p1; p += 32) t += partial[p];
    t = warp_sum(t);
    if (lane == 0) {
      eps[k] = eps_from_sumsq(t, prm);
      if (sumsq) sumsq[k] = t;
    }
  }
}

__global__ void __launch_bounds__(kThreads)
finalize_eps(const double *__restrict__ partial, int32_t nblocks, int32_t stride ,
             int32_t k0, int32_t ncolors_here, EpsParams prm, double *__restrict__ eps ,
             double *__restrict__ sumsq ) {
  const int lane = threadIdx.x & 31;
  const int c = (int)((blockIdx.x * (int64_t)kThreads + threadIdx.x) >> 5);
  if (c >= ncolors_here) return;
  double t = 0.0;
  for (int b = lane; b < nblocks; b += 32) t += partial[(int64_t)b * stride + c];
  t = warp_sum(t);
  if (lane == 0) {
    eps[k0 + c] = eps_from_sumsq(t, prm);
    if (sumsq) sumsq[k0 + c] = t;
  }
}

__global__ void __launch_bounds__(kThreads)
component_eps(const double *__restrict__ x, int64_t c0, int64_t ncols, int fdtype_central, double relstep,
              double absstep, double dir, double *__restrict__ eps) {
  const int64_t i = blockIdx.x * (int64_t)kThreads + threadIdx.x;
  if (i >= ncols) return;
  const double a = relstep * fabs(x[c0 + i]);
  double e = a > absstep ? a : absstep;
  if (!fdtype_central) e = e * dir;
  eps[i] = e;
}

}
```

finitediff.jl_b200/csrc/kernels_perturb.cuh:

```cuda
#pragma once
#include "common.cuh"

namespace fdb {

constexpr int kPerturbSmemColors = 1024;
constexpr int kPerturbMaxPoints = 4;

struct PerturbArgs {
  const double *x;
  const void *jcolor;
  const double *eps;
  double *xp, *xm;
  int64_t n, ldx;
  int32_t C, drift, kcount;
  int32_t k[kPerturbMaxPoints];
  int32_t aligned;
  int32_t reverse;
};

template <bool CENTRAL>
__device__ __forceinline__ void perturb_one(double v, uint32_t c, bool valid, double e, int drift, uint32_t k,
                                            double &p, double &q) {
  p = v;
  q = v;
  if (valid) {
    if (c == k) { p = v + e; if (CENTRAL) q = v - e; }
    else if (c < k && drift) { p = (v + e) - e; if (CENTRAL) q = (v - e) + e; }
  }
}

template <typename CT, bool CENTRAL, int NP>
__global__ void __launch_bounds__(kThreads)
perturb_colors(const PerturbArgs a) {
  extern __shared__ double s_eps[];
  const bool use_smem = a.C <= kPerturbSmemColors;
  if (use_smem) {
    for (int i = threadIdx.x; i < a.C; i += kThreads) s_eps[i] = a.eps[i];
    __syncthreads();
  }
  const CT *__restrict__ jcolor = reinterpret_cast<const CT *>(a.jcolor);
  constexpr int kHalf = kTile / 2;
  const int tid2 = 2 * threadIdx.x;
  const int64_t nfull = a.aligned ? a.n / kTile : 0;
  auto eps_of = [&](uint32_t c) -> double {
    return c < (uint32_t)a.C ? (use_smem ? s_eps[c] : __ldg(a.eps + c)) : 0.0;
  };
  for (int64_t pos = blockIdx.x; pos < nfull; pos += gridDim.x) {
    const int64_t base = (a.reverse ? nfull - 1 - pos : pos) * kTile;
    const double2 va = ld_stream2(a.x + base + tid2);
    const double2 vb = ld_stream2(a.x + base + kHalf + tid2);
    uint32_t ca0, ca1, cb0, cb1;
    ld_color_pair<CT>(jcolor + base + tid2, ca0, ca1);
    ld_color_pair<CT>(jcolor + base + kHalf + tid2, cb0, cb1);
    const double ea0 = eps_of(ca0), ea1 = eps_of(ca1), eb0 = eps_of(cb0), eb1 = eps_of(cb1);
    const bool ya0 = ca0 < (uint32_t)a.C, ya1 = ca1 < (uint32_t)a.C, yb0 = cb0 < (uint32_t)a.C, yb1 = cb1 < (uint32_t)a.C;
#pragma unroll
    for (int b = 0; b < NP; ++b) {
      if (NP > 1 && b >= a.kcount) break;
      const uint32_t k = (uint32_t)a.k[b];
      double p0, q0, p1, q1;
      perturb_one<CENTRAL>(va.x, ca0, ya0, ea0, a.drift, k, p0, q0);
      perturb_one<CENTRAL>(va.y, ca1, ya1, ea1, a.drift, k, p1, q1);
      st_stream2(a.xp + (int64_t)b * a.ldx + base + tid2, p0, p1);
      if (CENTRAL) st_stream2(a.xm + (int64_t)b * a.ldx + base + tid2, q0, q1);
      perturb_one<CENTRAL>(vb.x, cb0, yb0, eb0, a.drift, k, p0, q0);
      perturb_one<CENTRAL>(vb.y, cb1, yb1, eb1, a.drift, k, p1, q1);
      st_stream2(a.xp + (int64_t)b * a.ldx + base + kHalf + tid2, p0, p1);
      if (CENTRAL) st_stream2(a.xm + (int64_t)b * a.ldx + base + kHalf + tid2, q0, q1);
    }
  }
  const int64_t rem0 = nfull * kTile;
  const int64_t ntail = (a.n - rem0 + kTile - 1) / kTile;
  for (int64_t tt = blockIdx.x; tt < ntail; tt += gridDim.x) {
    for (int64_t j = rem0 + tt * kTile + threadIdx.x; j < a.n && j < rem0 + (tt + 1) * kTile; j += kThreads) {
      const double v = ld_stream(a.x + j);
      const uint32_t c = (uint32_t)jcolor[j];
      const bool y = c < (uint32_t)a.C;
      const double e = eps_of(c);
#pragma unroll
      for (int b = 0; b < NP; ++b) {
        if (NP > 1 && b >= a.kcount) break;
        double p, q;
        perturb_one<CENTRAL>(v, c, y, e, a.drift, (uint32_t)a.k[b], p, q);
        a.xp[(int64_t)b * a.ldx + j] = p;
        if (CENTRAL) a.xm[(int64_t)b * a.ldx + j] = q;
      }
    }
  }
}

template <typename CT, int NP>
__global__ void __launch_bounds__(kThreads)
perturb_complex(const PerturbArgs a) {
  const CT *__restrict__ jcolor = reinterpret_cast<const CT *>(a.jcolor);
  const int64_t stride = (int64_t)gridDim.x * kThreads;
  for (int64_t j = blockIdx.x * (int64_t)kThreads + threadIdx.x; j < a.n; j += stride) {
    const double v = ld_stream(a.x + j);
    const uint32_t c = (uint32_t)jcolor[j];
    const double e = c < (uint32_t)a.C ? __ldg(a.eps + c) : 0.0;
#pragma unroll
    for (int b = 0; b < NP; ++b) {
      if (NP > 1 && b >= a.kcount) break;
      st_stream2(a.xp + (int64_t)b * a.ldx + 2 * j, v, c == (uint32_t)a.k[b] ? e : 0.0);
    }
  }
}

__global__ void __launch_bounds__(kThreads)
replicate_x_complex(const double *__restrict__ x, int64_t n, int64_t ldx , int32_t B, double *__restrict__ X) {
  const int64_t stride = (int64_t)gridDim.x * kThreads;
  for (int64_t j = blockIdx.x * (int64_t)kThreads + threadIdx.x; j < n; j += stride) {
    const double v = x[j];
    for (int32_t b = 0; b < B; ++b) st_stream2(X + (int64_t)b * ldx + 2 * j, v, 0.0);
  }
}

__global__ void __launch_bounds__(kThreads)
set_components_complex(const double *__restrict__ eps_local, int64_t col0_local, int64_t c0, int64_t prev_c0, int32_t B,
                       int32_t prevB, int64_t ldx , double *__restrict__ X) {
  const int b = blockIdx.x * kThreads + threadIdx.x;
  if (b < prevB) X[(int64_t)b * ldx + 2 * (prev_c0 + b) + 1] = 0.0;
  if (b < B) X[(int64_t)b * ldx + 2 * (c0 + b) + 1] = eps_local[col0_local + b];
}

__global__ void __launch_bounds__(kThreads)
fill_value(double *__restrict__ p, int64_t n, double v) {
  const int64_t i = blockIdx.x * (int64_t)kThreads + threadIdx.x;
  if (i < n) p[i] = v;
}


__global__ void __launch_bounds__(kThreads)
replicate_x(const double *__restrict__ x, int64_t n, int64_t ldx, int32_t B, double *__restrict__ X) {
  const int64_t stride = (int64_t)gridDim.x * kThreads;
  for (int64_t j = blockIdx.x * (int64_t)kThreads + threadIdx.x; j < n; j += stride) {
    const double v = x[j];
    for (int32_t b = 0; b < B; ++b) X[(int64_t)b * ldx + j] = v;
  }
}

__global__ void __launch_bounds__(kThreads)
set_components(const double *__restrict__ x, const double *__restrict__ eps_local ,
               int64_t col0_local, int64_t c0, int64_t prev_c0, int32_t B, int32_t prevB, int64_t ldx, double sign,
               double *__restrict__ X) {
  const int b = blockIdx.x * kThreads + threadIdx.x;
  if (b < prevB) {
    const int64_t pc = prev_c0 + b;
    X[(int64_t)b * ldx + pc] = x[pc];
  }
  if (b < B) {
    const int64_t c = c0 + b;
    X[(int64_t)b * ldx + c] = x[c] + sign * eps_local[col0_local + b];
  }
}

}
```

finitediff.jl_b200/csrc/kernels_plan.cuh:

```cuda
#pragma once
#include "common.cuh"

namespace fdb {

enum PlanErr : uint32_t {
  kErrColptr = 1u,
  kErrRowRange = 2u,
  kErrColRange = 4u,
  kErrSlotRange = 8u,
  kErrPatternDiff = 16u,
  kErrMissingInJ = 32u,
  kErrRowOrder = 64u
};

__global__ void __launch_bounds__(kThreads)
color_minmax(const int64_t *__restrict__ colorvec, int64_t n, long long *__restrict__ out_max,
             long long *__restrict__ out_min) {
  long long mx = LLONG_MIN, mn = LLONG_MAX;
  const int64_t stride = (int64_t)gridDim.x * kThreads;
  for (int64_t j = blockIdx.x * (int64_t)kThreads + threadIdx.x; j < n; j += stride) {
    const long long c = colorvec[j];
    mx = c > mx ? c : mx;
    mn = c < mn ? c : mn;
  }
#pragma unroll
  for (int o = 16; o > 0; o >>= 1) {
    const long long a = __shfl_xor_sync(0xffffffffu, mx, o), b = __shfl_xor_sync(0xffffffffu, mn, o);
    mx = a > mx ? a : mx;
    mn = b < mn ? b : mn;
  }
  if ((threadIdx.x & 31) == 0) {
    atomicMax(out_max, mx);
    atomicMin(out_min, mn);
  }
}

template <typename CT>
__global__ void __launch_bounds__(kThreads)
convert_colors(const int64_t *__restrict__ colorvec , int64_t n, CT *__restrict__ jcolor) {
  const int64_t stride = (int64_t)gridDim.x * kThreads;
  for (int64_t j = blockIdx.x * (int64_t)kThreads + threadIdx.x; j < n; j += stride) {
    const int64_t c = colorvec ? colorvec[j] : j + 1;
    jcolor[j] = c >= 1 ? (CT)(c - 1) : (CT)ColorTraits<CT>::invalid;
  }
}

__global__ void __launch_bounds__(kThreads)
validate_colptr(const int64_t *__restrict__ colptr, int64_t n, int64_t nnz, uint32_t *__restrict__ err) {
  const int64_t stride = (int64_t)gridDim.x * kThreads;
  for (int64_t c = blockIdx.x * (int64_t)kThreads + threadIdx.x; c <= n; c += stride) {
    bool bad = false;
    if (c == 0 && colptr[0] != 1) bad = true;
    if (c == n && colptr[n] != nnz + 1) bad = true;
    if (c < n && colptr[c + 1] < colptr[c]) bad = true;
    if (bad) atomicOr(err, kErrColptr);
  }
}

__device__ __forceinline__ int64_t csc_col_of(const int64_t *__restrict__ colptr, int64_t n, int64_t p) {
  int64_t lo = 0, hi = n;
  while (hi - lo > 1) {
    const int64_t mid = (lo + hi) >> 1;
    if (colptr[mid] - 1 <= p) lo = mid; else hi = mid;
  }
  return lo;
}

constexpr int kPlanSmemColors = 4096;
__device__ __forceinline__ void count_color(uint32_t k, int32_t C, unsigned int *s_cnt ,
                                            unsigned long long *__restrict__ color_count) {
  const bool valid = k < (uint32_t)C;
  const unsigned act = __ballot_sync(0xffffffffu, valid);
  if (!valid) return;
  const unsigned peers = __match_any_sync(act, k);
  if ((int)(threadIdx.x & 31) != __ffs(peers) - 1) return;
  if (s_cnt) atomicAdd(s_cnt + k, (unsigned int)__popc(peers));
  else atomicAdd(color_count + k, (unsigned long long)__popc(peers));
}
__device__ __forceinline__ unsigned int *count_begin(unsigned int *smem, int32_t C, const unsigned long long *color_count) {
  if (color_count == nullptr || C > kPlanSmemColors) return nullptr;
  for (int i = threadIdx.x; i < C; i += kThreads) smem[i] = 0u;
  __syncthreads();
  return smem;
}
__device__ __forceinline__ void count_end(unsigned int *s_cnt, int32_t C, unsigned long long *__restrict__ color_count) {
  if (!s_cnt) return;
  __syncthreads();
  for (int i = threadIdx.x; i < C; i += kThreads)
    if (s_cnt[i]) atomicAdd(color_count + i, (unsigned long long)s_cnt[i]);
}

template <typename CT>
__global__ void __launch_bounds__(kThreads)
expand_csc(const int64_t *__restrict__ colptr, const int64_t *__restrict__ rowval, int64_t m, int64_t n, int64_t nnz,
           const CT *__restrict__ jcolor, int32_t C, int32_t *__restrict__ row32, CT *__restrict__ ecolor,
           int32_t *__restrict__ col32 , unsigned long long *__restrict__ color_count ,
           uint32_t *__restrict__ err) {
  extern __shared__ unsigned int s_hist[];
  unsigned int *s_cnt = count_begin(s_hist, C, color_count);
  const int64_t stride = (int64_t)gridDim.x * kThreads;
  const int lane = threadIdx.x & 31;
  for (int64_t p0 = blockIdx.x * (int64_t)kThreads + threadIdx.x - lane; p0 < nnz; p0 += stride) {
    const int64_t p = p0 + lane;
    uint32_t k = 0xffffffffu;
    if (p < nnz) {
      const int64_t c = csc_col_of(colptr, n, p);
      const int64_t r = rowval[p];
      if (r < 1 || r > m) { atomicOr(err, kErrRowRange); row32[p] = 0; }
      else row32[p] = (int32_t)(r - 1);
      if (p > colptr[c] - 1 && rowval[p - 1] >= r) atomicOr(err, kErrRowOrder);
      const CT kc = jcolor[c];
      ecolor[p] = kc;
      if (col32) col32[p] = (int32_t)c;
      k = (uint32_t)kc;
    }
    if (color_count) count_color(k, C, s_cnt, color_count);
  }
  count_end(s_cnt, C, color_count);
}

__global__ void __launch_bounds__(kThreads)
compare_i64(const int64_t *__restrict__ a, const int64_t *__restrict__ b, int64_t count, uint32_t *__restrict__ err) {
  const int64_t stride = (int64_t)gridDim.x * kThreads;
  bool diff = false;
  for (int64_t i = blockIdx.x * (int64_t)kThreads + threadIdx.x; i < count; i += stride) diff |= a[i] != b[i];
  if (diff) atomicOr(err, kErrPatternDiff);
}

__global__ void __launch_bounds__(kThreads)
dest_dense_from_rc(const int32_t *__restrict__ row32, const int32_t *__restrict__ col32, int64_t E, int64_t ldJ,
                   int64_t *__restrict__ dest) {
  const int64_t stride = (int64_t)gridDim.x * kThreads;
  for (int64_t e = blockIdx.x * (int64_t)kThreads + threadIdx.x; e < E; e += stride)
    dest[e] = (int64_t)col32[e] * ldJ + row32[e];
}

__global__ void __launch_bounds__(kThreads)
dest_other_csc(const int32_t *__restrict__ row32, const int32_t *__restrict__ col32, int64_t E,
               const int64_t *__restrict__ j_colptr, const int64_t *__restrict__ j_rowval, int64_t *__restrict__ dest,
               uint32_t *__restrict__ err) {
  const int64_t stride = (int64_t)gridDim.x * kThreads;
  for (int64_t e = blockIdx.x * (int64_t)kThreads + threadIdx.x; e < E; e += stride) {
    const int64_t c = col32[e], r = (int64_t)row32[e] + 1;
    int64_t lo = j_colptr[c] - 1, hi = j_colptr[c + 1] - 1;
    int64_t found = -1;
    while (lo < hi) {
      const int64_t mid = (lo + hi) >> 1;
      const int64_t rv = j_rowval[mid];
      if (rv == r) { found = mid; break; }
      if (rv < r) lo = mid + 1; else hi = mid;
    }
    if (found < 0) { atomicOr(err, kErrMissingInJ); found = 0; }
    dest[e] = found;
  }
}

template <typename CT>
__global__ void __launch_bounds__(kThreads)
prepare_coo(const int64_t *__restrict__ rows, const int64_t *__restrict__ cols, const int64_t *__restrict__ slots,
            int64_t nnz, int64_t m, int64_t n, int64_t ldJ, int64_t j_len, const CT *__restrict__ jcolor, int32_t C,
            int32_t *__restrict__ row32, CT *__restrict__ ecolor, int64_t *__restrict__ dest,
            unsigned long long *__restrict__ color_count, uint32_t *__restrict__ err) {
  extern __shared__ unsigned int s_hist[];
  unsigned int *s_cnt = count_begin(s_hist, C, color_count);
  const int64_t stride = (int64_t)gridDim.x * kThreads;
  const int lane = threadIdx.x & 31;
  for (int64_t e0 = blockIdx.x * (int64_t)kThreads + threadIdx.x - lane; e0 < nnz; e0 += stride) {
    const int64_t e = e0 + lane;
    uint32_t kk = 0xffffffffu;
    if (e < nnz) {
      int64_t r = rows[e], c = cols[e];
      if (r < 1 || r > m) { atomicOr(err, kErrRowRange); r = 1; }
      if (c < 1 || c > n) { atomicOr(err, kErrColRange); c = 1; }
      row32[e] = (int32_t)(r - 1);
      const CT k = jcolor[c - 1];
      ecolor[e] = k;
      int64_t d;
      if (slots) {
        d = slots[e] - 1;
        if (d < 0 || d >= j_len) { atomicOr(err, kErrSlotRange); d = 0; }
      } else {
        d = (c - 1) * ldJ + (r - 1);
      }
      dest[e] = d;
      kk = (uint32_t)k;
    }
    if (color_count) count_color(kk, C, s_cnt, color_count);
  }
  count_end(s_cnt, C, color_count);
}

template <typename CT>
__global__ void __launch_bounds__(kThreads)
colptr32_and_count(const int64_t *__restrict__ colptr, int64_t n, const CT *__restrict__ jcolor, int32_t C,
                   int32_t *__restrict__ colptr32, unsigned long long *__restrict__ bucket_count ) {
  const int64_t stride = (int64_t)gridDim.x * kThreads;
  for (int64_t c = blockIdx.x * (int64_t)kThreads + threadIdx.x; c <= n; c += stride) {
    colptr32[c] = (int32_t)(colptr[c] - 1);
    if (c < n) {
      uint32_t k = (uint32_t)jcolor[c];
      if (k >= (uint32_t)C) k = (uint32_t)C;
      const unsigned act = __activemask();
      const unsigned peers = __match_any_sync(act, k);
      if ((threadIdx.x & 31) == __ffs(peers) - 1) atomicAdd(bucket_count + k, (unsigned long long)__popc(peers));
    }
  }
}

template <typename CT>
__global__ void __launch_bounds__(kThreads)
count_color_buckets(const CT *__restrict__ jcolor, int64_t n, int32_t C, unsigned long long *__restrict__ bucket_count ) {
  const int64_t stride = (int64_t)gridDim.x * kThreads;
  for (int64_t c = blockIdx.x * (int64_t)kThreads + threadIdx.x; c < n; c += stride) {
    uint32_t k = (uint32_t)jcolor[c];
    if (k >= (uint32_t)C) k = (uint32_t)C;
    const unsigned act = __activemask();
    const unsigned peers = __match_any_sync(act, k);
    if ((threadIdx.x & 31) == __ffs(peers) - 1) atomicAdd(bucket_count + k, (unsigned long long)__popc(peers));
  }
}

template <typename CT>
__global__ void __launch_bounds__(kThreads)
color_sort_keys(const CT *__restrict__ jcolor, int64_t n, int32_t C, uint32_t *__restrict__ keys, int32_t *__restrict__ vals) {
  const int64_t stride = (int64_t)gridDim.x * kThreads;
  for (int64_t c = blockIdx.x * (int64_t)kThreads + threadIdx.x; c < n; c += stride) {
    uint32_t k = (uint32_t)jcolor[c];
    if (k >= (uint32_t)C) k = (uint32_t)C;
    keys[c] = k;
    vals[c] = (int32_t)c;
  }
}

__global__ void __launch_bounds__(kThreads)
cm_column_counts(const int32_t *__restrict__ list_cols, int64_t ncols, const int32_t *__restrict__ colptr32,
                 int32_t *__restrict__ list_cnt) {
  const int64_t stride = (int64_t)gridDim.x * kThreads;
  for (int64_t i = blockIdx.x * (int64_t)kThreads + threadIdx.x; i < ncols; i += stride) {
    const int32_t c = list_cols[i];
    list_cnt[i] = colptr32[c + 1] - colptr32[c];
  }
}

template <typename ST>
__global__ void __launch_bounds__(kThreads)
cm_expand(const int32_t *__restrict__ list_cols, const int32_t *__restrict__ list_off, int64_t ncols,
          const int32_t *__restrict__ colptr32, const int32_t *__restrict__ row32, const int64_t *__restrict__ dest,
          int lanes, int32_t *__restrict__ cm_row, ST *__restrict__ cm_slot) {
  const int cols_per_block = kThreads / lanes;
  const int sub = threadIdx.x % lanes;
  for (int64_t i = blockIdx.x * (int64_t)cols_per_block + threadIdx.x / lanes; i < ncols; i += (int64_t)gridDim.x * cols_per_block) {
    const int32_t c = list_cols[i];
    const int32_t p0 = colptr32[c], p1 = colptr32[c + 1];
    const int64_t q0 = list_off[i];
    for (int32_t p = p0 + sub; p < p1; p += lanes) {
      cm_row[q0 + (p - p0)] = row32[p];
      cm_slot[q0 + (p - p0)] = dest ? (ST)dest[p] : (ST)p;
    }
  }
}

template <typename CT>
__global__ void __launch_bounds__(kThreads)
color_lane_conflicts(const CT *__restrict__ jcolor, int64_t n, int32_t C, uint32_t *__restrict__ flags) {
  const int64_t stride = (int64_t)gridDim.x * kThreads;
  const int lane = threadIdx.x & 31;
  uint32_t bad = 0;
  for (int64_t c0 = blockIdx.x * (int64_t)kThreads + threadIdx.x - lane; c0 < n; c0 += stride) {
    const int64_t c = c0 + lane;
    const uint32_t k = c < n ? (uint32_t)jcolor[c] : 0xffffffffu;
    const bool valid = k < (uint32_t)C;
    const unsigned act = __ballot_sync(0xffffffffu, valid);
    if (!valid) continue;
    const unsigned others = __match_any_sync(act, k) & ~(1u << lane);
#pragma unroll
    for (int lg = 1; lg <= 5; ++lg) {
      const int g = 1 << lg;
      const unsigned group = (g == 32 ? 0xffffffffu : ((1u << g) - 1u)) << (lane & ~(g - 1));
      if (others & group) bad |= 1u << lg;
    }
  }
  if (bad) atomicOr(flags, bad);
}

__global__ void __launch_bounds__(kThreads)
row_jump_sum(const int32_t *__restrict__ row32, int64_t E, unsigned long long *__restrict__ out) {
  unsigned long long acc = 0;
  const int64_t stride = (int64_t)gridDim.x * kThreads;
  for (int64_t e = blockIdx.x * (int64_t)kThreads + threadIdx.x; e + 1 < E; e += stride) {
    long long d = (long long)row32[e + 1] - row32[e];
    if (d < 0) d = -d;
    acc += (unsigned long long)(d > (1 << 20) ? (1 << 20) : d);
  }
#pragma unroll
  for (int o = 16; o > 0; o >>= 1) acc += __shfl_xor_sync(0xffffffffu, acc, o);
  if ((threadIdx.x & 31) == 0) atomicAdd(out, acc);
}

template <typename CT>
__global__ void __launch_bounds__(kThreads)
count_band_colors(const CT *__restrict__ jcolor, int64_t m, int64_t n, int64_t l, int64_t u, int32_t C,
                  unsigned long long *__restrict__ color_count) {
  const int64_t stride = (int64_t)gridDim.x * kThreads;
  for (int64_t c = blockIdx.x * (int64_t)kThreads + threadIdx.x; c < n; c += stride) {
    const uint32_t k = (uint32_t)jcolor[c];
    if (k >= (uint32_t)C) continue;
    int64_t r_lo = c - u; if (r_lo < 0) r_lo = 0;
    int64_t r_hi = c + l; if (r_hi > m - 1) r_hi = m - 1;
    if (r_hi >= r_lo) atomicAdd(color_count + k, (unsigned long long)(r_hi - r_lo + 1));
  }
}

}
```

finitediff.jl_b200/csrc/kernels_staged.cuh:

```cuda
#pragma once
#include "common.cuh"
#include "kernels_scatter.cuh"

namespace fdb {

__device__ __forceinline__ uint32_t smem_u32(const void *p) { return (uint32_t)__cvta_generic_to_shared(p); }
__device__ __forceinline__ void mbar_init(uint64_t *bar, uint32_t count) {
  asm volatile("mbarrier.init.shared::cta.b64 [%0], %1;" ::"r"(smem_u32(bar)), "r"(count) : "memory");
}
__device__ __forceinline__ void mbar_arrive(uint64_t *bar) {
  asm volatile("mbarrier.arrive.shared::cta.b64 _, [%0];" ::"r"(smem_u32(bar)) : "memory");
}
__device__ __forceinline__ void mbar_arrive_expect_tx(uint64_t *bar, uint32_t bytes) {
  asm volatile("mbarrier.arrive.expect_tx.shared::cta.b64 _, [%0], %1;" ::"r"(smem_u32(bar)), "r"(bytes) : "memory");
}
__device__ __forceinline__ bool mbar_try_wait(uint64_t *bar, uint32_t parity) {
  uint32_t ok;
  asm volatile(
      "{\n\t.reg .pred p;\n\t"
      "mbarrier.try_wait.parity.shared::cta.b64 p, [%1], %2;\n\t"
      "selp.u32 %0, 1, 0, p;\n\t}"
      : "=r"(ok)
      : "r"(smem_u32(bar)), "r"(parity)
      : "memory");
  return ok != 0;
}
__device__ __forceinline__ void bulk_g2s(void *sdst, const void *gsrc, uint32_t bytes, uint64_t *bar) {
  asm volatile("cp.async.bulk.shared::cluster.global.mbarrier::complete_tx::bytes [%0], [%1], %2, [%3];" ::"r"(smem_u32(sdst)),
               "l"(__cvta_generic_to_global(gsrc)), "r"(bytes), "r"(smem_u32(bar))
               : "memory");
}
__device__ __forceinline__ void fence_mbar_init() {
  asm volatile("fence.mbarrier_init.release.cluster;" ::: "memory");
  asm volatile("fence.proxy.async.shared::cta;" ::: "memory");
}

constexpr int kStageMaxWin = 8;
constexpr int kStagesMax = 3;
constexpr int kStageMaxSmem = 46 * 1024;

struct StagedArgs {
  const uint16_t *row16;
  const void *ecolor;
  const int32_t *tile_w0;
  const int32_t *row32;
  const double *fx, *Fp, *Fm, *eps;
  double *J;
  int32_t C, W;
  int32_t stages;
  int64_t ldF, src_len;
  int64_t E;
  int32_t j_aligned;
  int32_t reverse;
};

template <typename CT>
__global__ void __launch_bounds__(kThreads)
stage_prepare(const int32_t *__restrict__ row32, int64_t ntiles, int32_t *__restrict__ tile_w0, uint16_t *__restrict__ row16,
              unsigned int *__restrict__ max_span, const CT *__restrict__ ecolor ,
              int32_t C) {
  __shared__ int32_t s_min[kThreads / 32], s_max[kThreads / 32];
  __shared__ int32_t s_w0;
  for (int64_t tile = blockIdx.x; tile < ntiles; tile += gridDim.x) {
    const int32_t *rt = row32 + tile * kTile;
    int32_t r[kTile / kThreads];
    int32_t mn = INT_MAX, mx = INT_MIN;
#pragma unroll
    for (int u = 0; u < kTile / kThreads; ++u) {
      r[u] = rt[u * kThreads + threadIdx.x];
      mn = min(mn, r[u]);
      mx = max(mx, r[u]);
    }
#pragma unroll
    for (int o = 16; o > 0; o >>= 1) {
      mn = min(mn, __shfl_xor_sync(0xffffffffu, mn, o));
      mx = max(mx, __shfl_xor_sync(0xffffffffu, mx, o));
    }
    if ((threadIdx.x & 31) == 0) { s_min[threadIdx.x >> 5] = mn; s_max[threadIdx.x >> 5] = mx; }
    __syncthreads();
    if (threadIdx.x == 0) {
      int32_t a = s_min[0], b = s_max[0];
      for (int w = 1; w < kThreads / 32; ++w) { a = min(a, s_min[w]); b = max(b, s_max[w]); }
      a &= ~1;
      s_w0 = a;
      tile_w0[tile] = a;
      atomicMax(max_span, (unsigned int)(b - a + 1));
    }
    __syncthreads();
    const int32_t w0 = s_w0;
#pragma unroll
    for (int u = 0; u < kTile / kThreads; ++u) {
      int32_t d = r[u] - w0;
      d = d > 65535 ? 65535 : d;
      if (ecolor) {
        uint32_t k = (uint32_t)ecolor[tile * kTile + u * kThreads + threadIdx.x];
        if (k >= (uint32_t)C) k = 15u;
        d = (d & 0xFFF) | (int32_t)(k << 12);
      }
      row16[tile * kTile + u * kThreads + threadIdx.x] = (uint16_t)d;
    }
    __syncthreads();
  }
}

template <typename CT, int MODE, int MINB, bool PREFETCH, bool PACKED, bool EMPTYBAR = false>
__global__ void __launch_bounds__(kThreads, MINB)
diff_scatter_staged(const StagedArgs a) {
  static_assert(MODE == kForward || MODE == kCentral, "staged scatter: forward / central");
  extern __shared__ __align__(128) unsigned char smem_raw[];
  const int C = a.C, W = a.W;
  const int nwin = MODE == kCentral ? 2 * C : C + 1;
  const int stage_elems = nwin * W;
  const int kStages = a.stages;
  double *buf = reinterpret_cast<double *>(smem_raw);
  uint64_t *full = reinterpret_cast<uint64_t *>(buf + kStages * stage_elems);
  uint64_t *empty = full + kStagesMax;
  double *s_eps = reinterpret_cast<double *>(full + 2 * kStagesMax);
  const CT *__restrict__ ecolor = reinterpret_cast<const CT *>(a.ecolor);
  const int64_t nfull = a.E / kTile;
  constexpr int kHalf = kTile / 2;
  const int tid2 = 2 * threadIdx.x;
  auto phys = [&](int64_t t) -> int64_t { return a.reverse ? nfull - 1 - t : t; };

  auto issue = [&](int64_t tile, int s) {
    const int32_t w0 = __ldg(a.tile_w0 + tile);
    int64_t len = a.src_len - w0;
    if (len > W) len = W;
    const uint32_t bytes = (uint32_t)len * 8u;
    double *dst = buf + s * stage_elems;
    mbar_arrive_expect_tx(full + s, bytes * (uint32_t)nwin);
    for (int k = 0; k < C; ++k) bulk_g2s(dst + k * W, a.Fp + (int64_t)k * a.ldF + w0, bytes, full + s);
    if (MODE == kCentral) {
      for (int k = 0; k < C; ++k) bulk_g2s(dst + (C + k) * W, a.Fm + (int64_t)k * a.ldF + w0, bytes, full + s);
    } else {
      bulk_g2s(dst + C * W, a.fx + w0, bytes, full + s);
    }
  };

  if (threadIdx.x == 0) {
    for (int s = 0; s < kStages; ++s) { mbar_init(full + s, 1); mbar_init(empty + s, kThreads / 32); }
    fence_mbar_init();
  }
  for (int i = threadIdx.x; i < C; i += kThreads) s_eps[i] = a.eps[i];
  __syncthreads();
  if (threadIdx.x == 0) {
    for (int s = 0; s < kStages; ++s) {
      const int64_t t = (int64_t)blockIdx.x + (int64_t)s * gridDim.x;
      if (t < nfull) issue(phys(t), s);
    }
  }

  auto value = [&](const double *__restrict__ win, uint32_t r, uint32_t k) -> double {
    if (k >= (uint32_t)C) return 0.0;
    const double e = s_eps[k];
    const double hi = win[k * W + r];
    const double lo = MODE == kCentral ? win[(C + k) * W + r] : win[C * W + r];
    const double d = hi - lo;
    return d / (MODE == kCentral ? 2 * e : e);
  };

  struct Idx { ushort2 ra, rb; uint32_t ka0, ka1, kb0, kb1; };
  auto load_idx = [&](int64_t tile) {
    Idx x;
    const uint16_t *__restrict__ rt = a.row16 + tile * kTile;
    const CT *__restrict__ ct = ecolor + tile * kTile;
    x.ra = __ldcs(reinterpret_cast<const ushort2 *>(rt + tid2));
    x.rb = __ldcs(reinterpret_cast<const ushort2 *>(rt + kHalf + tid2));
    if (PACKED) {
      x.ka0 = x.ra.x >> 12; x.ka1 = x.ra.y >> 12; x.kb0 = x.rb.x >> 12; x.kb1 = x.rb.y >> 12;
      x.ra.x &= 0xFFF; x.ra.y &= 0xFFF; x.rb.x &= 0xFFF; x.rb.y &= 0xFFF;
    } else {
      ld_color_pair<CT>(ct + tid2, x.ka0, x.ka1);
      ld_color_pair<CT>(ct + kHalf + tid2, x.kb0, x.kb1);
    }
    return x;
  };
  uint32_t it = 0;
  int s = 0;
  uint32_t parity = 0;
  Idx nx{};
  if (PREFETCH && (int64_t)blockIdx.x < nfull) nx = load_idx(phys(blockIdx.x));
  for (int64_t pos = blockIdx.x; pos < nfull; pos += gridDim.x, ++it) {
    const int64_t tile = phys(pos);
    double *__restrict__ Jt = a.J + tile * kTile;
    const Idx cur = PREFETCH ? nx : load_idx(tile);
    if (PREFETCH && pos + gridDim.x < nfull) nx = load_idx(phys(pos + gridDim.x));
    const ushort2 ra = cur.ra, rb = cur.rb;
    const uint32_t ka0 = cur.ka0, ka1 = cur.ka1, kb0 = cur.kb0, kb1 = cur.kb1;
    while (!mbar_try_wait(full + s, parity)) {}
    const double *__restrict__ win = buf + s * stage_elems;
    const double va0 = value(win, ra.x, ka0), va1 = value(win, ra.y, ka1);
    const double vb0 = value(win, rb.x, kb0), vb1 = value(win, rb.y, kb1);
    if (a.j_aligned) {
      st_stream2(Jt + tid2, va0, va1);
      st_stream2(Jt + kHalf + tid2, vb0, vb1);
    } else {
      Jt[tid2] = va0; Jt[tid2 + 1] = va1; Jt[kHalf + tid2] = vb0; Jt[kHalf + tid2 + 1] = vb1;
    }
    if (EMPTYBAR) {
      __syncwarp();
      if ((threadIdx.x & 31) == 0) mbar_arrive(empty + s);
      if (threadIdx.x == 0) {
        const int64_t nxt = pos + (int64_t)kStages * gridDim.x;
        if (nxt < nfull) {
          while (!mbar_try_wait(empty + s, parity)) {}
          issue(phys(nxt), s);
        }
      }
    } else {
      __syncthreads();
      if (threadIdx.x == 0) {
        const int64_t nxt = pos + (int64_t)kStages * gridDim.x;
        if (nxt < nfull) issue(phys(nxt), s);
      }
    }
    if (++s == kStages) { s = 0; parity ^= 1u; }
  }
  const int64_t rem0 = nfull * kTile;
  if (rem0 < a.E && blockIdx.x == (unsigned)(nfull % gridDim.x)) {
    for (int64_t e = rem0 + threadIdx.x; e < a.E; e += kThreads) {
      const uint32_t k = (uint32_t)ecolor[e];
      double v = 0.0;
      if (k < (uint32_t)C)
        v = fd_quotient<MODE>(a.Fp + (int64_t)k * a.ldF, MODE == kCentral ? a.Fm + (int64_t)k * a.ldF : a.fx, a.row32[e], s_eps[k]);
      a.J[e] = v;
    }
  }
}

}
```

Before: 48.67 billion.

## Derive banded row indices and cyclic colours arithmetically instead of loading index streams

```diff
diff --git a/finitediff.jl_b200/csrc/common.cuh b/finitediff.jl_b200/csrc/common.cuh
--- a/finitediff.jl_b200/csrc/common.cuh
+++ b/finitediff.jl_b200/csrc/common.cuh
@@ -35,6 +35,49 @@
   a = (uint32_t)v.x; b = (uint32_t)v.y;
 }
 
+struct FastDiv {
+  uint32_t d, magic, s1, s2;
+  __device__ __forceinline__ uint32_t div(uint32_t j) const {
+    const uint32_t t = __umulhi(j, magic);
+    return (t + ((j - t) >> s1)) >> s2;
+  }
+  __device__ __forceinline__ uint32_t mod(uint32_t j) const { return j - div(j) * d; }
+};
+inline FastDiv make_fastdiv(uint32_t d) {
+  uint32_t l = 0;
+  while ((1ull << l) < d) ++l;
+  FastDiv f;
+  f.d = d;
+  f.magic = (uint32_t)(((1ull << 32) * ((1ull << l) - d)) / d + 1);
+  f.s1 = l > 0 ? 1 : 0;
+  f.s2 = l > 0 ? l - 1 : 0;
+  return f;
+}
+
+template <typename CT> struct TableColors {
+  const CT *p;
+  __device__ __forceinline__ uint32_t at(int64_t j) const { return (uint32_t)__ldg(p + j); }
+  __device__ __forceinline__ void tile(int64_t base, int tid2, uint32_t &a0, uint32_t &a1, uint32_t &b0, uint32_t &b1) const {
+    ld_color_pair<CT>(p + base + tid2, a0, a1);
+    ld_color_pair<CT>(p + base + kTile / 2 + tid2, b0, b1);
+  }
+};
+struct CyclicColors {
+  FastDiv P;
+  __device__ __forceinline__ uint32_t at(int64_t j) const { return P.mod((uint32_t)j); }
+  __device__ __forceinline__ uint32_t plus(uint32_t a, uint32_t b) const {
+    const uint32_t s = a + b;
+    return s >= P.d ? s - P.d : s;
+  }
+  __device__ __forceinline__ void tile(int64_t base, int tid2, uint32_t &a0, uint32_t &a1, uint32_t &b0, uint32_t &b1) const {
+    const uint32_t b = P.mod((uint32_t)base);
+    a0 = plus(b, P.mod((uint32_t)tid2));
+    a1 = plus(a0, 1u);
+    b0 = plus(b, P.mod((uint32_t)(kTile / 2 + tid2)));
+    b1 = plus(b0, 1u);
+  }
+};
+
 __device__ __forceinline__ double warp_sum(double v) {
 #pragma unroll
   for (int o = 16; o > 0; o >>= 1) v += __shfl_xor_sync(0xffffffffu, v, o);
diff --git a/finitediff.jl_b200/csrc/fdjac_abi.cu b/finitediff.jl_b200/csrc/fdjac_abi.cu
--- a/finitediff.jl_b200/csrc/fdjac_abi.cu
+++ b/finitediff.jl_b200/csrc/fdjac_abi.cu
@@ -94,6 +94,7 @@
   int32_t C = 0;
   int color_bits = 8;
   bool has_invalid = false;
+  bool cyclic = false;
   void *jcolor = nullptr;
   int32_t *row32 = nullptr;
   void *ecolor = nullptr;
@@ -121,7 +122,7 @@
   bool lists_resident = false;
   struct Tunables {
     bool no_staged = false, no_eps_lists = false, no_eps_overlap = false, cm_prefetch = false, force_overlap = false;
-    bool no_fx_cm = false, force_fx_cm = false, no_pack = false;
+    bool no_fx_cm = false, force_fx_cm = false, no_pack = false, no_band = false;
     int hi_stream = -1;
     int reverse = 3;
     int cm_slab_stream = 1;
@@ -145,6 +146,8 @@
   int32_t *tile_w0 = nullptr;
   int32_t stage_W = 0;
   bool staged = false, stage_packed = false;
+  bool stage_band = false;
+  int32_t band_l = 0, band_col_a = 0, band_col_b = 0, band_e_a = 0, band_e_b = 0, band_w = 1;
   std::vector<int64_t> bucket_start;
   int lanes = 1;
   double mean_row_jump = 0.0;
@@ -230,6 +233,11 @@
   return fn((int32_t)0);
 }
 
+template <typename CT, typename F> static fdb_status dispatch_colors(const fdb_plan *P, F &&fn) {
+  if (P->cyclic) return fn(CyclicColors{make_fastdiv((uint32_t)P->C)});
+  return fn(TableColors<CT>{(const CT *)P->jcolor});
+}
+
 static const char *plan_err_text(uint32_t e) {
   if (e & kErrColptr) return "colptr is not a valid CSC column pointer (must start at 1, be non-decreasing, end at nnz+1)";
   if (e & kErrRowRange) return "row index outside 1..m";
@@ -266,25 +274,27 @@
   if (n > 0) {
     uint32_t *d_flags = nullptr;
     const bool window_path = P->C > kEpsRegColors;
-    if (window_path) {
-      CU(cudaMalloc((void **)&d_flags, sizeof(uint32_t)));
-      CU(cudaMemset(d_flags, 0, sizeof(uint32_t)));
-    }
+    CU(cudaMalloc((void **)&d_flags, 2 * sizeof(uint32_t)));
+    CU(cudaMemset(d_flags, 0, 2 * sizeof(uint32_t)));
     fdb_status st = dispatch_ct(P->color_bits, [&](auto tag) -> fdb_status {
       using CT = decltype(tag);
       convert_colors<CT><<<P->grid(n), kThreads>>>(cv.d, n, (CT *)P->jcolor);
       if (window_path) color_lane_conflicts<CT><<<P->grid(n), kThreads>>>((const CT *)P->jcolor, n, P->C, d_flags);
+      if (P->C > 0) check_cyclic<CT><<<P->grid(n), kThreads>>>((const CT *)P->jcolor, n, P->C, d_flags + 1);
       CU(cudaGetLastError());
       return FDB_OK;
     });
-    if (st == FDB_OK && window_path) {
-      uint32_t flags = 0;
-      cudaError_t e = cudaMemcpy(&flags, d_flags, sizeof flags, cudaMemcpyDeviceToHost);
-      if (e != cudaSuccess) st = fail(FDB_ERR_CUDA, "colour conflict flags: %s", cudaGetErrorString(e));
-      P->eps_group = 1;
-      for (int lg = 1; lg <= 5 && !(flags & (1u << lg)); ++lg) P->eps_group = 1 << lg;
-    }
-    if (d_flags) cudaFree(d_flags);
+    if (st == FDB_OK) {
+      uint32_t flags[2] = {0, 0};
+      cudaError_t e = cudaMemcpy(flags, d_flags, sizeof flags, cudaMemcpyDeviceToHost);
+      if (e != cudaSuccess) st = fail(FDB_ERR_CUDA, "colour flags: %s", cudaGetErrorString(e));
+      P->cyclic = P->C > 0 && flags[1] == 0;
+      if (window_path) {
+        P->eps_group = 1;
+        for (int lg = 1; lg <= 5 && !(flags[0] & (1u << lg)); ++lg) P->eps_group = 1 << lg;
+      }
+    }
+    cudaFree(d_flags);
     if (st != FDB_OK) return st;
   }
   return FDB_OK;
@@ -528,6 +538,38 @@
   return FDB_OK;
 }
 
+static fdb_status try_band_form(fdb_plan *P) {
+  P->stage_band = false;
+  const int64_t m = P->m, n = P->n;
+  int *d_lu = nullptr;
+  uint32_t *d_flag = nullptr;
+  TRY(P->alloc_t(&d_lu, 2));
+  TRY(P->alloc_t(&d_flag, 1));
+  const int init[2] = {INT_MIN, INT_MIN};
+  CU(cudaMemcpy(d_lu, init, sizeof init, cudaMemcpyHostToDevice));
+  CU(cudaMemset(d_flag, 0, 4));
+  band_extent<<<P->grid(n), kThreads>>>(P->colptr32, P->row32, n, d_lu);
+  int lu[2];
+  CU(cudaMemcpy(lu, d_lu, sizeof lu, cudaMemcpyDeviceToHost));
+  const int l = lu[0], u = lu[1];
+  band_check<<<P->grid(n), kThreads>>>(P->colptr32, P->row32, m, n, l, u, d_flag);
+  uint32_t bad = 1;
+  CU(cudaMemcpy(&bad, d_flag, 4, cudaMemcpyDeviceToHost));
+  if (bad) return FDB_OK;
+  const int64_t a = std::min<int64_t>(std::max(l, 0), n), b = std::max<int64_t>(a, std::min<int64_t>(n, m - u));
+  int32_t ea = 0, eb = 0;
+  CU(cudaMemcpy(&ea, P->colptr32 + a, 4, cudaMemcpyDeviceToHost));
+  CU(cudaMemcpy(&eb, P->colptr32 + b, 4, cudaMemcpyDeviceToHost));
+  P->band_l = l;
+  P->band_w = l + u + 1;
+  P->band_col_a = (int32_t)a;
+  P->band_col_b = (int32_t)b;
+  P->band_e_a = ea;
+  P->band_e_b = eb;
+  P->stage_band = true;
+  return FDB_OK;
+}
+
 static fdb_status try_stage_plan(fdb_plan *P) {
   P->staged = false;
   if (P->tune.no_staged) return FDB_OK;
@@ -560,6 +602,7 @@
   if (span == 0 || span > 65535 || smem > (size_t)kStageMaxSmem) return FDB_OK;
   P->stage_W = (int32_t)W;
   P->staged = true;
+  if (!P->tune.no_band) TRY(try_band_form(P));
   return FDB_OK;
 }
 
@@ -587,6 +630,7 @@
   t.no_fx_cm = env_is("FDB_NO_FX_CM", '1');
   t.force_fx_cm = env_is("FDB_FORCE_FX_CM", '1');
   t.no_pack = env_is("FDB_NO_PACK", '1');
+  t.no_band = env_is("FDB_NO_BAND", '1');
   if (const char *hs = getenv("FDB_HI_STREAM")) t.hi_stream = hs[0] == '1' ? 1 : 0;
   if (const char *v = getenv("FDB_REVERSE")) { if (v[0] >= '0' && v[0] <= '3') t.reverse = v[0] - '0'; }
   if (env_is("FDB_CM_HINT", '0')) t.cm_slab_stream = 0;
@@ -1042,8 +1086,11 @@
         const int64_t C = std::max<int32_t>(P->C, 1);
         const int64_t owned = P->world > 1 ? P->E * (int64_t)P->local_colors.size() / C : P->E;
         info->moved_bytes_scatter = P->E * (4 + ct) * std::max<int64_t>(P->n_groups, 1) + owned * (8 * slabs_read + 8 + (P->dest ? 8 : 0)) + fx_once;
-        if (P->staged)
-          info->moved_bytes_scatter = P->E * (2 + (P->stage_packed ? 0 : ct) + 8) + 8 * P->m * (int64_t)(P->fdtype == FDB_CENTRAL ? 2 * P->C : P->C + 1);
+        const int64_t staged_rows = 8 * P->m * (int64_t)(P->fdtype == FDB_CENTRAL ? 2 * P->C : P->C + 1);
+        if (P->staged && P->stage_band)
+          info->moved_bytes_scatter = 8 * P->E + staged_rows + (P->cyclic ? 0 : P->n * ct);
+        else if (P->staged)
+          info->moved_bytes_scatter = P->E * (2 + (P->stage_packed ? 0 : ct) + 8) + staged_rows;
       }
     } else {
       info->moved_bytes_scatter = P->alg_bytes;
@@ -1203,12 +1250,16 @@
   if (C <= kEpsRegColors) {
     const int64_t ntiles = (P->n + kTile - 1) / kTile;
     const int aligned = (reinterpret_cast<uintptr_t>(x) & 15) == 0;
-    auto go = [&](auto kern) {
-      const int grid = std::min(resident_grid(P, kern, 0, ntiles), P->eps_blocks);
-      kern<<<grid, kThreads, 0, s>>>(x, (const CT *)P->jcolor, P->n, aligned, C, prm, P->partial, P->ticket, P->eps, P->sumsq);
-    };
-    if (C <= 4) { if (P->tune.eps_depth == 2) go(color_sumsq_reg<CT, 4, 2>); else go(color_sumsq_reg<CT, 4, 1>); }
-    else { if (P->tune.eps_depth == 2) go(color_sumsq_reg<CT, 8, 2>); else go(color_sumsq_reg<CT, 8, 1>); }
+    TRY(dispatch_colors<CT>(P, [&](auto cs) -> fdb_status {
+      using CS = decltype(cs);
+      auto go = [&](auto kern) {
+        const int grid = std::min(resident_grid(P, kern, 0, ntiles), P->eps_blocks);
+        kern<<<grid, kThreads, 0, s>>>(x, cs, P->n, aligned, C, prm, P->partial, P->ticket, P->eps, P->sumsq);
+      };
+      if (C <= 4) { if (P->tune.eps_depth == 2) go(color_sumsq_reg<CS, 4, 2>); else go(color_sumsq_reg<CS, 4, 1>); }
+      else { if (P->tune.eps_depth == 2) go(color_sumsq_reg<CS, 8, 2>); else go(color_sumsq_reg<CS, 8, 1>); }
+      return FDB_OK;
+    }));
     P->cnt.kernel_launches += 1;
   } else {
     for (int32_t k0 = 0; k0 < C; k0 += kEpsWindow) {
@@ -1265,7 +1316,7 @@
   auto perturb_window = [&](int64_t li0, int64_t kc) -> fdb_status {
       for (int64_t q0 = 0; q0 < kc; q0 += kPerturbMaxPoints) {
         PerturbArgs pa{};
-        pa.x = x; pa.jcolor = P->jcolor; pa.eps = P->eps;
+        pa.x = x; pa.eps = P->eps;
         pa.xp = P->xp + q0 * sX; pa.xm = CENTRAL ? P->xm + q0 * sX : nullptr;
         pa.n = P->n; pa.ldx = sX; pa.C = P->C; pa.drift = P->no_drift ? 0 : 1;
         pa.reverse = (P->tune.reverse >> 1) & 1;
@@ -1275,17 +1326,21 @@
                        reinterpret_cast<uintptr_t>(P->xm)) & 15) == 0 && (P->ldx & 1) == 0;
         const size_t sm = P->C <= kPerturbSmemColors ? (size_t)P->C * sizeof(double) : 0;
         const int64_t tiles = (P->n + kTile - 1) / kTile;
-        if (COMPLEX) {
-          if (pa.kcount == 1) perturb_complex<CT, 1><<<P->grid(P->n), kThreads, 0, s>>>(pa);
-          else perturb_complex<CT, kPerturbMaxPoints><<<P->grid(P->n), kThreads, 0, s>>>(pa);
-        } else {
-          constexpr int kPerturbGridOver = 16;
-          auto over = [&](int g) { return (int)std::max<int64_t>(1, std::min<int64_t>((int64_t)g * kPerturbGridOver, tiles)); };
-          if (pa.kcount == 1)
-            perturb_colors<CT, CENTRAL, 1><<<over(resident_grid(P, perturb_colors<CT, CENTRAL, 1>, sm, tiles)), kThreads, sm, s>>>(pa);
-          else
-            perturb_colors<CT, CENTRAL, kPerturbMaxPoints><<<over(resident_grid(P, perturb_colors<CT, CENTRAL, kPerturbMaxPoints>, sm, tiles)), kThreads, sm, s>>>(pa);
-        }
+        TRY(dispatch_colors<CT>(P, [&](auto cs) -> fdb_status {
+          using CS = decltype(cs);
+          if (COMPLEX) {
+            if (pa.kcount == 1) perturb_complex<CS, 1><<<P->grid(P->n), kThreads, 0, s>>>(pa, cs);
+            else perturb_complex<CS, kPerturbMaxPoints><<<P->grid(P->n), kThreads, 0, s>>>(pa, cs);
+          } else {
+            constexpr int kPerturbGridOver = 16;
+            auto over = [&](int g) { return (int)std::max<int64_t>(1, std::min<int64_t>((int64_t)g * kPerturbGridOver, tiles)); };
+            if (pa.kcount == 1)
+              perturb_colors<CS, CENTRAL, 1><<<over(resident_grid(P, perturb_colors<CS, CENTRAL, 1>, sm, tiles)), kThreads, sm, s>>>(pa, cs);
+            else
+              perturb_colors<CS, CENTRAL, kPerturbMaxPoints><<<over(resident_grid(P, perturb_colors<CS, CENTRAL, kPerturbMaxPoints>, sm, tiles)), kThreads, sm, s>>>(pa, cs);
+          }
+          return FDB_OK;
+        }));
         P->cnt.kernel_launches += 1;
       }
       return FDB_OK;
@@ -1399,25 +1454,40 @@
         if (staged) {
           if constexpr (MODE != kComplex) {
             StagedArgs sa{};
-            sa.row16 = P->row16; sa.ecolor = P->ecolor; sa.tile_w0 = P->tile_w0; sa.row32 = P->row32;
+            sa.row16 = P->row16; sa.tile_w0 = P->tile_w0; sa.row32 = P->row32;
             sa.fx = vfx; sa.Fp = P->Fp; sa.Fm = P->Fm; sa.eps = P->eps; sa.J = J; sa.C = P->C; sa.W = P->stage_W;
             sa.ldF = sF; sa.src_len = P->ldF; sa.E = P->E; sa.j_aligned = a.j_aligned;
             sa.reverse = P->tune.reverse & 1;
+            sa.colptr32 = P->colptr32; sa.l = P->band_l; sa.n = (int32_t)P->n;
+            sa.col_a = P->band_col_a; sa.col_b = P->band_col_b; sa.e_a = P->band_e_a; sa.e_b = P->band_e_b;
+            sa.w = make_fastdiv((uint32_t)P->band_w);
             const int nwin = CENTRAL ? 2 * P->C : P->C + 1;
             int stages = P->tune.stages;
             if ((size_t)stages * nwin * P->stage_W * 8 + 2 * kStagesMax * 8 + (size_t)P->C * 8 > (size_t)kStageMaxSmem) stages = 2;
             sa.stages = stages;
             const size_t ssm = (size_t)stages * nwin * P->stage_W * 8 + 2 * kStagesMax * 8 + (size_t)P->C * 8;
             const char v0 = P->tune.staged_variant[0], v1 = P->tune.staged_variant[1];
-            auto go = [&](auto kern) {
+            auto go = [&](auto kern, auto cs) {
               const int grid = resident_grid(P, kern, ssm, tiles);
-              kern<<<grid, kThreads, ssm, s>>>(sa);
+              kern<<<grid, kThreads, ssm, s>>>(sa, cs);
             };
-            if (P->stage_packed && v1 == 'e') go(diff_scatter_staged<CT, MODE, 6, false, true, true>);
-            else if (P->stage_packed) go(diff_scatter_staged<CT, MODE, 6, false, true>);
-            else if (v0 == '8') go(diff_scatter_staged<CT, MODE, 8, false, false>);
-            else if (v1 == 'n') go(diff_scatter_staged<CT, MODE, 6, false, false>);
-            else go(diff_scatter_staged<CT, MODE, 6, true, false>);
+            if (P->stage_band) {
+              TRY(dispatch_colors<CT>(P, [&](auto cs) -> fdb_status {
+                using CS = decltype(cs);
+                if (v0 == '8') go(diff_scatter_staged<CS, MODE, 8, false, false, false, true>, cs);
+                else if (v1 == 'e') go(diff_scatter_staged<CS, MODE, 6, false, false, true, true>, cs);
+                else go(diff_scatter_staged<CS, MODE, 6, false, false, false, true>, cs);
+                return FDB_OK;
+              }));
+            } else {
+              using CS = TableColors<CT>;
+              const CS ec{(const CT *)P->ecolor};
+              if (P->stage_packed && v1 == 'e') go(diff_scatter_staged<CS, MODE, 6, false, true, true>, ec);
+              else if (P->stage_packed) go(diff_scatter_staged<CS, MODE, 6, false, true>, ec);
+              else if (v0 == '8') go(diff_scatter_staged<CS, MODE, 8, false, false>, ec);
+              else if (v1 == 'n') go(diff_scatter_staged<CS, MODE, 6, false, false>, ec);
+              else go(diff_scatter_staged<CS, MODE, 6, true, false>, ec);
+            }
           }
         } else if (full) {
           const int grid = resident_grid(P, diff_scatter_ident<CT, MODE, true, kScatterMinBlocks>, sm, tiles);
diff --git a/finitediff.jl_b200/csrc/kernels_eps.cuh b/finitediff.jl_b200/csrc/kernels_eps.cuh
--- a/finitediff.jl_b200/csrc/kernels_eps.cuh
+++ b/finitediff.jl_b200/csrc/kernels_eps.cuh
@@ -29,9 +29,9 @@
     if (c == (uint32_t)k) acc[k] += sq;
 }
 
-template <typename CT, int NC, int DEPTH = 1>
-__global__ void __launch_bounds__(kThreads)
-color_sumsq_reg(const double *__restrict__ x, const CT *__restrict__ jcolor, int64_t n, int x_aligned, int32_t C,
+template <typename CS, int NC, int DEPTH = 1>
+__global__ void __launch_bounds__(kThreads)
+color_sumsq_reg(const double *__restrict__ x, const CS colors, int64_t n, int x_aligned, int32_t C,
                 EpsParams prm, double *__restrict__ partial ,
                 unsigned int *__restrict__ ticket, double *__restrict__ eps, double *__restrict__ sumsq) {
   double acc[NC];
@@ -44,14 +44,11 @@
   if (DEPTH == 2) {
     for (; tile + gridDim.x < nfull; tile += 2 * (int64_t)gridDim.x) {
       const double *__restrict__ xa = x + tile * kTile, *__restrict__ xb = xa + (int64_t)gridDim.x * kTile;
-      const CT *__restrict__ ca = jcolor + tile * kTile, *__restrict__ cb = ca + (int64_t)gridDim.x * kTile;
       const double2 a0 = ld_stream2(xa + tid2), a1 = ld_stream2(xa + kHalf + tid2);
       const double2 b0 = ld_stream2(xb + tid2), b1 = ld_stream2(xb + kHalf + tid2);
       uint32_t p0, p1, p2, p3, q0, q1, q2, q3;
-      ld_color_pair<CT>(ca + tid2, p0, p1);
-      ld_color_pair<CT>(ca + kHalf + tid2, p2, p3);
-      ld_color_pair<CT>(cb + tid2, q0, q1);
-      ld_color_pair<CT>(cb + kHalf + tid2, q2, q3);
+      colors.tile(tile * kTile, tid2, p0, p1, p2, p3);
+      colors.tile((tile + gridDim.x) * kTile, tid2, q0, q1, q2, q3);
       sumsq_accumulate<NC>(acc, a0.x, p0);
       sumsq_accumulate<NC>(acc, a0.y, p1);
       sumsq_accumulate<NC>(acc, a1.x, p2);
@@ -64,12 +61,10 @@
   }
   for (; tile < nfull; tile += gridDim.x) {
     const double *__restrict__ xt = x + tile * kTile;
-    const CT *__restrict__ ct = jcolor + tile * kTile;
     const double2 va = ld_stream2(xt + tid2);
     const double2 vb = ld_stream2(xt + kHalf + tid2);
     uint32_t ca0, ca1, cb0, cb1;
-    ld_color_pair<CT>(ct + tid2, ca0, ca1);
-    ld_color_pair<CT>(ct + kHalf + tid2, cb0, cb1);
+    colors.tile(tile * kTile, tid2, ca0, ca1, cb0, cb1);
     sumsq_accumulate<NC>(acc, va.x, ca0);
     sumsq_accumulate<NC>(acc, va.y, ca1);
     sumsq_accumulate<NC>(acc, vb.x, cb0);
@@ -83,8 +78,8 @@
 #pragma unroll
       for (int u = 0; u < kPairsPerThread; ++u) {
         const int64_t j = base + u * kHalf + tid2;
-        if (j < n) sumsq_accumulate<NC>(acc, ld_stream(x + j), (uint32_t)jcolor[j]);
-        if (j + 1 < n) sumsq_accumulate<NC>(acc, ld_stream(x + j + 1), (uint32_t)jcolor[j + 1]);
+        if (j < n) sumsq_accumulate<NC>(acc, ld_stream(x + j), colors.at(j));
+        if (j + 1 < n) sumsq_accumulate<NC>(acc, ld_stream(x + j + 1), colors.at(j + 1));
       }
     }
   }
diff --git a/finitediff.jl_b200/csrc/kernels_perturb.cuh b/finitediff.jl_b200/csrc/kernels_perturb.cuh
--- a/finitediff.jl_b200/csrc/kernels_perturb.cuh
+++ b/finitediff.jl_b200/csrc/kernels_perturb.cuh
@@ -8,7 +8,6 @@
 
 struct PerturbArgs {
   const double *x;
-  const void *jcolor;
   const double *eps;
   double *xp, *xm;
   int64_t n, ldx;
@@ -29,16 +28,15 @@
   }
 }
 
-template <typename CT, bool CENTRAL, int NP>
+template <typename CS, bool CENTRAL, int NP>
 __global__ void __launch_bounds__(kThreads)
-perturb_colors(const PerturbArgs a) {
+perturb_colors(const PerturbArgs a, const CS colors) {
   extern __shared__ double s_eps[];
   const bool use_smem = a.C <= kPerturbSmemColors;
   if (use_smem) {
     for (int i = threadIdx.x; i < a.C; i += kThreads) s_eps[i] = a.eps[i];
     __syncthreads();
   }
-  const CT *__restrict__ jcolor = reinterpret_cast<const CT *>(a.jcolor);
   constexpr int kHalf = kTile / 2;
   const int tid2 = 2 * threadIdx.x;
   const int64_t nfull = a.aligned ? a.n / kTile : 0;
@@ -50,8 +48,7 @@
     const double2 va = ld_stream2(a.x + base + tid2);
     const double2 vb = ld_stream2(a.x + base + kHalf + tid2);
     uint32_t ca0, ca1, cb0, cb1;
-    ld_color_pair<CT>(jcolor + base + tid2, ca0, ca1);
-    ld_color_pair<CT>(jcolor + base + kHalf + tid2, cb0, cb1);
+    colors.tile(base, tid2, ca0, ca1, cb0, cb1);
     const double ea0 = eps_of(ca0), ea1 = eps_of(ca1), eb0 = eps_of(cb0), eb1 = eps_of(cb1);
     const bool ya0 = ca0 < (uint32_t)a.C, ya1 = ca1 < (uint32_t)a.C, yb0 = cb0 < (uint32_t)a.C, yb1 = cb1 < (uint32_t)a.C;
 #pragma unroll
@@ -74,7 +71,7 @@
   for (int64_t tt = blockIdx.x; tt < ntail; tt += gridDim.x) {
     for (int64_t j = rem0 + tt * kTile + threadIdx.x; j < a.n && j < rem0 + (tt + 1) * kTile; j += kThreads) {
       const double v = ld_stream(a.x + j);
-      const uint32_t c = (uint32_t)jcolor[j];
+      const uint32_t c = colors.at(j);
       const bool y = c < (uint32_t)a.C;
       const double e = eps_of(c);
 #pragma unroll
@@ -89,14 +86,13 @@
   }
 }
 
-template <typename CT, int NP>
+template <typename CS, int NP>
 __global__ void __launch_bounds__(kThreads)
-perturb_complex(const PerturbArgs a) {
-  const CT *__restrict__ jcolor = reinterpret_cast<const CT *>(a.jcolor);
+perturb_complex(const PerturbArgs a, const CS colors) {
   const int64_t stride = (int64_t)gridDim.x * kThreads;
   for (int64_t j = blockIdx.x * (int64_t)kThreads + threadIdx.x; j < a.n; j += stride) {
     const double v = ld_stream(a.x + j);
-    const uint32_t c = (uint32_t)jcolor[j];
+    const uint32_t c = colors.at(j);
     const double e = c < (uint32_t)a.C ? __ldg(a.eps + c) : 0.0;
 #pragma unroll
     for (int b = 0; b < NP; ++b) {
diff --git a/finitediff.jl_b200/csrc/kernels_plan.cuh b/finitediff.jl_b200/csrc/kernels_plan.cuh
--- a/finitediff.jl_b200/csrc/kernels_plan.cuh
+++ b/finitediff.jl_b200/csrc/kernels_plan.cuh
@@ -42,6 +42,50 @@
   for (int64_t j = blockIdx.x * (int64_t)kThreads + threadIdx.x; j < n; j += stride) {
     const int64_t c = colorvec ? colorvec[j] : j + 1;
     jcolor[j] = c >= 1 ? (CT)(c - 1) : (CT)ColorTraits<CT>::invalid;
+  }
+}
+
+template <typename CT>
+__global__ void __launch_bounds__(kThreads)
+check_cyclic(const CT *__restrict__ jcolor, int64_t n, int32_t C, uint32_t *__restrict__ flag) {
+  const int64_t stride = (int64_t)gridDim.x * kThreads;
+  for (int64_t j = blockIdx.x * (int64_t)kThreads + threadIdx.x; j < n; j += stride)
+    if ((uint32_t)jcolor[j] != (uint32_t)(j % C)) { *flag = 1u; return; }
+}
+
+__global__ void __launch_bounds__(kThreads)
+band_extent(const int32_t *__restrict__ colptr32, const int32_t *__restrict__ row32, int64_t n, int *__restrict__ lu) {
+  int l = INT_MIN, u = INT_MIN;
+  const int64_t stride = (int64_t)gridDim.x * kThreads;
+  for (int64_t c = blockIdx.x * (int64_t)kThreads + threadIdx.x; c < n; c += stride) {
+    const int32_t p0 = colptr32[c], p1 = colptr32[c + 1];
+    if (p1 > p0) {
+      for (int32_t p = p0; p < p1; ++p) {
+        const int r = row32[p];
+        l = max(l, (int)c - r);
+        u = max(u, r - (int)c);
+      }
+    }
+  }
+#pragma unroll
+  for (int o = 16; o > 0; o >>= 1) {
+    l = max(l, __shfl_xor_sync(0xffffffffu, l, o));
+    u = max(u, __shfl_xor_sync(0xffffffffu, u, o));
+  }
+  if ((threadIdx.x & 31) == 0) { atomicMax(lu, l); atomicMax(lu + 1, u); }
+}
+
+__global__ void __launch_bounds__(kThreads)
+band_check(const int32_t *__restrict__ colptr32, const int32_t *__restrict__ row32, int64_t m, int64_t n, int l, int u,
+           uint32_t *__restrict__ flag) {
+  const int64_t stride = (int64_t)gridDim.x * kThreads;
+  for (int64_t c = blockIdx.x * (int64_t)kThreads + threadIdx.x; c < n; c += stride) {
+    const int64_t lo = c - l > 0 ? c - l : 0, hi = c + u < m - 1 ? c + u : m - 1;
+    const int64_t len = hi >= lo ? hi - lo + 1 : 0;
+    const int32_t p0 = colptr32[c];
+    bool bad = colptr32[c + 1] - p0 != len;
+    for (int64_t i = 0; !bad && i < len; ++i) bad = row32[p0 + i] != lo + i;
+    if (bad) { *flag = 1u; return; }
   }
 }
 
diff --git a/finitediff.jl_b200/csrc/kernels_staged.cuh b/finitediff.jl_b200/csrc/kernels_staged.cuh
--- a/finitediff.jl_b200/csrc/kernels_staged.cuh
+++ b/finitediff.jl_b200/csrc/kernels_staged.cuh
@@ -41,7 +41,6 @@
 
 struct StagedArgs {
   const uint16_t *row16;
-  const void *ecolor;
   const int32_t *tile_w0;
   const int32_t *row32;
   const double *fx, *Fp, *Fm, *eps;
@@ -52,7 +51,28 @@
   int64_t E;
   int32_t j_aligned;
   int32_t reverse;
+  const int32_t *colptr32;
+  int32_t l, n;
+  int32_t col_a, col_b;
+  int32_t e_a, e_b;
+  FastDiv w;
 };
+
+__device__ __forceinline__ void band_locate(const StagedArgs &a, uint32_t e, uint32_t &c, uint32_t &r) {
+  if (e >= (uint32_t)a.e_a && e < (uint32_t)a.e_b) {
+    const uint32_t q = a.w.div(e - a.e_a);
+    c = a.col_a + q;
+    r = c - a.l + (e - a.e_a - q * a.w.d);
+    return;
+  }
+  int32_t lo = e < (uint32_t)a.e_a ? 0 : a.col_b, hi = e < (uint32_t)a.e_a ? a.col_a : a.n;
+  while (hi - lo > 1) {
+    const int32_t mid = (lo + hi) >> 1;
+    if ((uint32_t)__ldg(a.colptr32 + mid) <= e) lo = mid; else hi = mid;
+  }
+  c = (uint32_t)lo;
+  r = (uint32_t)max(0, lo - a.l) + (e - (uint32_t)__ldg(a.colptr32 + lo));
+}
 
 template <typename CT>
 __global__ void __launch_bounds__(kThreads)
@@ -103,10 +123,11 @@
   }
 }
 
-template <typename CT, int MODE, int MINB, bool PREFETCH, bool PACKED, bool EMPTYBAR = false>
+template <typename CS, int MODE, int MINB, bool PREFETCH, bool PACKED, bool EMPTYBAR = false, bool BAND = false>
 __global__ void __launch_bounds__(kThreads, MINB)
-diff_scatter_staged(const StagedArgs a) {
+diff_scatter_staged(const StagedArgs a, const CS colors) {
   static_assert(MODE == kForward || MODE == kCentral, "staged scatter: forward / central");
+  static_assert(!(BAND && (PACKED || PREFETCH)), "band form: no index stream to pack or prefetch");
   extern __shared__ __align__(128) unsigned char smem_raw[];
   const int C = a.C, W = a.W;
   const int nwin = MODE == kCentral ? 2 * C : C + 1;
@@ -116,7 +137,6 @@
   uint64_t *full = reinterpret_cast<uint64_t *>(buf + kStages * stage_elems);
   uint64_t *empty = full + kStagesMax;
   double *s_eps = reinterpret_cast<double *>(full + 2 * kStagesMax);
-  const CT *__restrict__ ecolor = reinterpret_cast<const CT *>(a.ecolor);
   const int64_t nfull = a.E / kTile;
   constexpr int kHalf = kTile / 2;
   const int tid2 = 2 * threadIdx.x;
@@ -162,16 +182,39 @@
   struct Idx { ushort2 ra, rb; uint32_t ka0, ka1, kb0, kb1; };
   auto load_idx = [&](int64_t tile) {
     Idx x;
-    const uint16_t *__restrict__ rt = a.row16 + tile * kTile;
-    const CT *__restrict__ ct = ecolor + tile * kTile;
-    x.ra = __ldcs(reinterpret_cast<const ushort2 *>(rt + tid2));
-    x.rb = __ldcs(reinterpret_cast<const ushort2 *>(rt + kHalf + tid2));
-    if (PACKED) {
-      x.ka0 = x.ra.x >> 12; x.ka1 = x.ra.y >> 12; x.kb0 = x.rb.x >> 12; x.kb1 = x.rb.y >> 12;
-      x.ra.x &= 0xFFF; x.ra.y &= 0xFFF; x.rb.x &= 0xFFF; x.rb.y &= 0xFFF;
-    } else {
-      ld_color_pair<CT>(ct + tid2, x.ka0, x.ka1);
-      ld_color_pair<CT>(ct + kHalf + tid2, x.kb0, x.kb1);
+    if constexpr (BAND) {
+      const uint32_t e0 = (uint32_t)(tile * kTile), w0 = (uint32_t)__ldg(a.tile_w0 + tile);
+      const bool interior = e0 >= (uint32_t)a.e_a && e0 + kTile <= (uint32_t)a.e_b;
+      auto pair = [&](uint32_t e, ushort2 &rr, uint32_t &k0, uint32_t &k1) {
+        uint32_t c, r, c1, r1;
+        if (interior) {
+          const uint32_t v = e - a.e_a, q = a.w.div(v), o = v - q * a.w.d;
+          c = a.col_a + q;
+          r = c - a.l + o;
+          const bool wrap = o + 1 == a.w.d;
+          c1 = wrap ? c + 1 : c;
+          r1 = wrap ? c1 - a.l : r + 1;
+        } else {
+          band_locate(a, e, c, r);
+          band_locate(a, e + 1, c1, r1);
+        }
+        rr.x = (unsigned short)(r - w0);
+        rr.y = (unsigned short)(r1 - w0);
+        k0 = colors.at(c);
+        k1 = c1 == c ? k0 : colors.at(c1);
+      };
+      pair(e0 + tid2, x.ra, x.ka0, x.ka1);
+      pair(e0 + kHalf + tid2, x.rb, x.kb0, x.kb1);
+    } else {
+      const uint16_t *__restrict__ rt = a.row16 + tile * kTile;
+      x.ra = __ldcs(reinterpret_cast<const ushort2 *>(rt + tid2));
+      x.rb = __ldcs(reinterpret_cast<const ushort2 *>(rt + kHalf + tid2));
+      if (PACKED) {
+        x.ka0 = x.ra.x >> 12; x.ka1 = x.ra.y >> 12; x.kb0 = x.rb.x >> 12; x.kb1 = x.rb.y >> 12;
+        x.ra.x &= 0xFFF; x.ra.y &= 0xFFF; x.rb.x &= 0xFFF; x.rb.y &= 0xFFF;
+      } else {
+        colors.tile(tile * kTile, tid2, x.ka0, x.ka1, x.kb0, x.kb1);
+      }
     }
     return x;
   };
@@ -219,10 +262,18 @@
   const int64_t rem0 = nfull * kTile;
   if (rem0 < a.E && blockIdx.x == (unsigned)(nfull % gridDim.x)) {
     for (int64_t e = rem0 + threadIdx.x; e < a.E; e += kThreads) {
-      const uint32_t k = (uint32_t)ecolor[e];
+      uint32_t k, r;
+      if constexpr (BAND) {
+        uint32_t c;
+        band_locate(a, (uint32_t)e, c, r);
+        k = colors.at(c);
+      } else {
+        k = colors.at(e);
+        r = (uint32_t)a.row32[e];
+      }
       double v = 0.0;
       if (k < (uint32_t)C)
-        v = fd_quotient<MODE>(a.Fp + (int64_t)k * a.ldF, MODE == kCentral ? a.Fm + (int64_t)k * a.ldF : a.fx, a.row32[e], s_eps[k]);
+        v = fd_quotient<MODE>(a.Fp + (int64_t)k * a.ldF, MODE == kCentral ? a.Fm + (int64_t)k * a.ldF : a.fx, r, s_eps[k]);
       a.J[e] = v;
     }
   }
```

Result: faster. 50.14 billion (median of 6 runs) (+3.0%).
